# BurryChen/lv_slam

Hardware: AMD Instinct MI355X
Metric: NDT registrations/sec (64k-pt Velodyne pairs) (higher is better)
Workload: dtype f32 terms, f64 accumulation

## Files before the change

lv_slam_amd/csrc/ndt_async.hpp:

```cpp
#pragma once
#include "ndt_types.hpp"
#include "ndt_math.hpp"
#include "ndt_sweep.hpp"
#include "ndt_update.hpp"
#include "ndt_pose_record.hpp"

#define ASYNC_POS_STRIDE 32
#define ASYNC_ARR_STRIDE 16
#define ASYNC_MAX_CTX    4
#define ASYNC_MAX_CARRY  128
#define ASYNC_CTX_SHIFT  24

struct AsyncCtx {
  const float* src; size_t pitch;
  PairState* st; const GridDesc* gd; const BitWord* words; const VoxelRec* recs; const float* cent;
  double* partials; const int* src_cnt; unsigned* arrived; mi355ndt_result* results;
  unsigned* n_done;
  int must_finish;
  int pose_base; PoseRecord* pose; int pose_stride;
  int score_only;
};
struct AsyncTab { AsyncCtx c[ASYNC_MAX_CTX]; };
#define NDT_GP(T) __attribute__((address_space(1))) T*
struct AsyncCtxG {
  NDT_GP(const float) src; size_t pitch;
  NDT_GP(PairState) st; NDT_GP(const GridDesc) gd; NDT_GP(const BitWord) words; NDT_GP(const VoxelRec) recs; NDT_GP(const float) cent;
  NDT_GP(double) partials; NDT_GP(const int) src_cnt; NDT_GP(unsigned) arrived; NDT_GP(mi355ndt_result) results;
  NDT_GP(unsigned) n_done;
  int must_finish;
  int pose_base; NDT_GP(PoseRecord) pose; int pose_stride, score_only;
};
static_assert(sizeof(AsyncCtxG) == sizeof(AsyncCtx) && offsetof(AsyncCtxG, pose) == offsetof(AsyncCtx, pose) && offsetof(AsyncCtxG, n_done) == offsetof(AsyncCtx, n_done),
              "AsyncCtxG mirrors AsyncCtx");
__device__ __forceinline__ AsyncCtx async_ctx_load(const AsyncTab* __restrict__ tab, const int ci) {
  const AsyncCtxG& g = reinterpret_cast<const AsyncCtxG*>(tab->c)[ci];
  AsyncCtx c;
  c.src = (const float*)g.src; c.pitch = g.pitch; c.st = (PairState*)g.st; c.gd = (const GridDesc*)g.gd; c.words = (const BitWord*)g.words;
  c.recs = (const VoxelRec*)g.recs; c.cent = (const float*)g.cent; c.partials = (double*)g.partials; c.src_cnt = (const int*)g.src_cnt;
  c.arrived = (unsigned*)g.arrived; c.results = (mi355ndt_result*)g.results; c.n_done = (unsigned*)g.n_done; c.must_finish = g.must_finish;
  c.pose_base = g.pose_base; c.pose = (PoseRecord*)g.pose; c.pose_stride = g.pose_stride; c.score_only = g.score_only;
  return c;
}
struct CtxStat { unsigned done, total_words, max_cells, plan_exceeded; };
struct StreamStatus { unsigned fin, abort_, n_live, susp; CtxStat ctx[ASYNC_MAX_CTX]; unsigned seq; unsigned pad0_;
                      unsigned long long build_t0, build_t1;
                      unsigned pad_[6]; };
static_assert(sizeof(StreamStatus) == 128, "one status slot is 128 bytes");

struct AsyncCtl {
  unsigned pub;
  unsigned fin;
  unsigned abort_;
  unsigned n_live;
  unsigned susp;
  unsigned pad_[27];
  unsigned pos[8 * ASYNC_POS_STRIDE];
  unsigned carry[ASYNC_MAX_CARRY];
};

#ifndef ASYNC_CLAIM
#define ASYNC_CLAIM(K) ((K) == 1 ? 2 : 1)
#endif
#ifndef ASYNC_HELP_RINGS
#define ASYNC_HELP_RINGS 1
#endif
#define ASYNC_HELP_AFTER 64u
#define ASYNC_SPIN_LIMIT (1u << 18)

NDT_KERNEL void k_async_prepare(const AsyncTab tab, AsyncTab* tab_dev, const int new_ci, const int n_new, PairState* st, const float* __restrict__ guess_cm,
                                const int* __restrict__ src_cnt, const GridDesc* __restrict__ gd, unsigned* arrived, int* active_list, SweepCtl* sweep_ctl ,
                                int* ring, const int ring_cap, AsyncCtl* ctl, const AsyncCtl* prev, unsigned* done_new ,
                                PoseRecord* pose_new , const int pose_cap, unsigned long long* stamp ) {
  const size_t i = (size_t)blockIdx.x * blockDim.x + threadIdx.x;
  if (i == 0 && stamp) *stamp = (unsigned long long)wall_clock64();
  const unsigned nc = prev ? min(prev->susp, (unsigned)ASYNC_MAX_CARRY) : 0u;
  const unsigned n_live = nc + (unsigned)n_new;
  if (i < (size_t)8 * ring_cap) {
    const size_t g = (i % (size_t)ring_cap) * 8 + i / (size_t)ring_cap;
    int w = -1;
    if (g < nc) w = (int)prev->carry[g];
    else if (g < n_live) w = (new_ci << ASYNC_CTX_SHIFT) | (int)(g - nc);
    ring[i] = w;
  }
  if (i < (size_t)n_new * ASYNC_ARR_STRIDE) arrived[i] = 0u;
  if (i < offsetof(AsyncCtl, carry) / sizeof(unsigned)) reinterpret_cast<unsigned*>(ctl)[i] = (i == 0 || i == 3) ? n_live : 0u;
  if (sweep_ctl && i < 2 * sizeof(SweepCtl) / sizeof(int)) reinterpret_cast<int*>(sweep_ctl)[i] = i == 0 ? n_new : 0;
  if (i == 0 && done_new && n_new > 0) *done_new = 0u;
  if (pose_new && i < (size_t)pose_cap) pose_new[i] = pose_record_padding();
  if (i == 0) tab_dev->c[0] = tab.c[0];
  if (i == 1) tab_dev->c[1] = tab.c[1];
  if (i == 2) tab_dev->c[2] = tab.c[2];
  if (i == 3) tab_dev->c[3] = tab.c[3];
  static_assert(ASYNC_MAX_CTX == 4, "the table is copied entry by entry");
  if (i < (size_t)n_new) {
    if (active_list) active_list[i] = (int)i;
    init_pair_state(st[i], guess_cm + i * 16, src_cnt[i], gd[i].status);
  }
}

__device__ __forceinline__ void async_update(const AsyncCtx& C, const int b, const int tw, const int n_pts, const int rows_per_pair, PairState& Ssh, volatile double* sol,
                                             int* ring, const int ring_cap, AsyncCtl* ctl, const unsigned n_live, const int stop_thresh, unsigned long long* hits_total,
                                             const double step_max, const double eps, const int max_iterations, Timeline& tl) {
  PairState* st = C.st;
  const double* partials = C.partials;
  mi355ndt_result* results = C.results;
  const int lane = threadIdx.x & 63;
  __builtin_amdgcn_s_setprio(3);
  gu64* sg = (gu64*)reinterpret_cast<unsigned long long*>(&st[b]);
  unsigned long long* sl = reinterpret_cast<unsigned long long*>(&Ssh);
  state_to_lds<true>(Ssh, &st[b], lane, 64);
  if (lane == 0) sol[6] = 0.0;
  const int nchunks = (n_pts + CHUNK_PTS - 1) / CHUNK_PTS;
  double aw[UPD_WAVES] = {0.0, 0.0, 0.0, 0.0};
  if (lane < NACC) walk_groups<4, true, 2, UPD_WAVES>(partials + (size_t)b * rows_per_pair * NACC + lane, nchunks, 0, 1, aw);
  wave_lds_sync();
  const bool last = __builtin_amdgcn_readfirstlane(Ssh.last_sweep) != 0;
  store_sums(Ssh, lane, wave_sums_total(aw[0], aw[1], aw[2], aw[3]), false, last, hits_total);
  wave_lds_sync();
  TL_STAMP(12);
  constexpr int RB0 = (int)(offsetof(PairState, reb_pn) / 8), RBT = (int)(offsetof(PairState, reb_tag) / 8);
  static_assert(RBT - RB0 == 14, "6 + 8 words of re-basing");
  const bool want_reb = Ssh.phase == PH_STEP;
  bool reb_ok = want_reb && Ssh.reb_tag == (long long)Ssh.sweeps;
  unsigned long long rbw = 0;
  if (reb_ok && lane < 14) rbw = __hip_atomic_load(sg + RB0 + lane, RLX_AGENT);
  if (!last) newton_solve_side(Ssh, sol);
  else if (lane == 0) {
    for (int a = 0; a < 6; a++) sol[a] = 0.0;
    sol[6] = 1.0;
  }
  wave_lds_sync();
  TL_STAMP(13);
  if (want_reb && !reb_ok) {
    unsigned spins = 0;
    while (!reb_ok && spins++ < (1u << 16)) {
      __builtin_amdgcn_s_sleep(2);
      long long tg = 0;
      if (lane == 0) tg = (long long)__hip_atomic_load(sg + RBT, RLX_AGENT);
      reb_ok = __shfl(tg, 0) == (long long)Ssh.sweeps;
    }
    if (reb_ok && lane < 14) rbw = __hip_atomic_load(sg + RB0 + lane, RLX_AGENT);
  }
  if (reb_ok && lane < 14) sl[RB0 + lane] = rbw;
  wave_lds_sync();
  const bool rebased = reb_ok;
  int rc = newton_update(Ssh, &results[b], step_max, eps, max_iterations, 0, sol, rebased, C.score_only != 0);
  rc = __builtin_amdgcn_readfirstlane(rc);
  wave_lds_sync();
  TL_STAMP(14);
  state_from_lds<true>(&st[b], Ssh, lane, 64);
  asm volatile("s_waitcnt vmcnt(0)" ::: "memory");
  if (lane == 0) {
    bool suspend = false;
    if (rc == NEWTON_SWEEP && stop_thresh > 0 && !C.must_finish)
      suspend = n_live - __hip_atomic_load((const gu32*)&ctl->fin, RLX_AGENT) <= (unsigned)stop_thresh;
    if (rc == NEWTON_SWEEP && !suspend) {
      const unsigned g = __hip_atomic_fetch_add((gu32*)&ctl->pub, 1u, RLX_AGENT);
      __hip_atomic_store((gu32*)reinterpret_cast<unsigned*>(ring + (size_t)(g & 7u) * ring_cap + (g >> 3)), (unsigned)tw, RLX_AGENT);
    } else if (rc == NEWTON_SWEEP) {
      const unsigned k = __hip_atomic_fetch_add((gu32*)&ctl->susp, 1u, RLX_AGENT);
      if (k < (unsigned)ASYNC_MAX_CARRY) __hip_atomic_store((gu32*)&ctl->carry[k], (unsigned)tw, RLX_AGENT);
      asm volatile("s_waitcnt vmcnt(0)" ::: "memory");
      __hip_atomic_fetch_add((gu32*)&ctl->fin, 1u, RLX_AGENT);
    } else {
      if (C.pose) C.pose[b] = pose_record(Ssh.final_cm, Ssh.score, Ssh.it, Ssh.converged, C.pose_base + b * C.pose_stride);
      asm volatile("s_waitcnt vmcnt(0)" ::: "memory");
      if (C.n_done) __hip_atomic_fetch_add((gu32*)C.n_done, 1u, RLX_AGENT);
      __hip_atomic_fetch_add((gu32*)&ctl->fin, 1u, RLX_AGENT);
    }
  }
  TL_STAMP(9);
  if (rc == NEWTON_SWEEP) {
    constexpr int RBI = (int)(offsetof(PairState, reb_inc) / 8);
    double pn[6]; float inc[16];
    newton_rebase(Ssh.p, Ssh.dir, Ssh.a_t, pn, inc);
    if (lane == 0) {
      for (int a = 0; a < 6; a++) __hip_atomic_store(sg + RB0 + a, (unsigned long long)__double_as_longlong(pn[a]), RLX_AGENT);
      for (int a = 0; a < 8; a++)
        __hip_atomic_store(sg + RBI + a, (unsigned long long)__float_as_uint(inc[2 * a]) | ((unsigned long long)__float_as_uint(inc[2 * a + 1]) << 32), RLX_AGENT);
      asm volatile("s_waitcnt vmcnt(0)" ::: "memory");
      __hip_atomic_store(sg + RBT, (unsigned long long)(long long)Ssh.sweeps, RLX_AGENT);
    }
  }
  __builtin_amdgcn_s_setprio(0);
}

NDT_KERNEL void k_stream_inputs(const unsigned* __restrict__ host_in, unsigned* __restrict__ dev_in, const unsigned n_in, unsigned* __restrict__ clear, const unsigned n_clear,
                                unsigned long long* stamp) {
  if (threadIdx.x == 0 && stamp) *stamp = (unsigned long long)wall_clock64();
  for (unsigned i = threadIdx.x; i < n_in; i += blockDim.x) dev_in[i] = host_in[i];
  for (unsigned i = threadIdx.x; i < n_clear; i += blockDim.x) clear[i] = 0u;
}

NDT_KERNEL void k_stream_status(const AsyncCtl* __restrict__ ctl, const CtxStat* __restrict__ stat, volatile unsigned* host_slot, const unsigned seq) {
  const int i = threadIdx.x;
  static_assert(offsetof(AsyncCtl, fin) == 4 && offsetof(AsyncCtl, susp) == 16 && offsetof(StreamStatus, ctx) == 16 && offsetof(StreamStatus, seq) == 80 && offsetof(StreamStatus, build_t0) == 88, "status layout");
  if (i < 4) host_slot[i] = reinterpret_cast<const unsigned*>(ctl)[1 + i];
  else if (i < 4 + 4 * ASYNC_MAX_CTX) host_slot[i] = reinterpret_cast<const unsigned*>(stat)[i - 4];
  __threadfence_system();
  __syncthreads();
  if (i == 0) host_slot[20] = seq;
}

#define NDT_CTX_PARAMS(i) const float* __restrict__ src##i, size_t pitch##i, PairState* st##i, const GridDesc* __restrict__ gd##i, const BitWord* __restrict__ words##i, \
                          const VoxelRec* __restrict__ recs##i, double* partials##i, const int* __restrict__ src_cnt##i, unsigned* arrived##i, const float* __restrict__ cent##i
#define NDT_CTX_SEL(f, ci) ((ci) == 0 ? f##0 : (ci) == 1 ? f##1 : (ci) == 2 ? f##2 : f##3)
template <bool PCA, int K, int ORD, bool LEAN = false>
__global__ void __launch_bounds__(SWEEP_THREADS, (SweepTune<PCA, K, ORD, LEAN>::WPE))
k_align_async(const AsyncTab* __restrict__ tab, int items_per_pair, int* ring, int ring_cap, AsyncCtl* ctl, SweepConst sc, unsigned long long* hits_total,
              double step_max, double eps, int max_iterations, int stop_thresh, unsigned debug_abort_pos, unsigned debug_ring_mask, int claim_items,
              NDT_CTX_PARAMS(0), NDT_CTX_PARAMS(1), NDT_CTX_PARAMS(2), NDT_CTX_PARAMS(3)) {
  const int lane = threadIdx.x & 63, wv = threadIdx.x >> 6;
  __shared__ double exp_tab[64];
  __shared__ PairState Ssh[WAVES];
  __shared__ double sol[WAVES][SOL_WORDS];
  if (threadIdx.x < 64) exp_tab[threadIdx.x] = ndtm::c_exp2_64[threadIdx.x];
  __syncthreads();
  const int x = blockIdx.x & 7;
  if (!((debug_ring_mask >> x) & 1u)) return;
  const gu32* ringx = (const gu32*)reinterpret_cast<const unsigned*>(ring + (size_t)x * ring_cap);
  const gu32* fin_p = (const gu32*)&ctl->fin;
  gu32* pos_p = (gu32*)&ctl->pos[x * ASYNC_POS_STRIDE];
  const unsigned n_live = ctl->n_live;
  const int I = items_per_pair;
  const int CLAIM = K == 1 ? ASYNC_CLAIM(1) : (claim_items == 2 ? 2 : 1);
  const int Iu = I / CLAIM;
  Timeline tl;
  auto give_up = [&]() {
    __hip_atomic_store((gu32*)&ctl->abort_, 1u, RLX_AGENT);
    __hip_atomic_store((gu32*)&ctl->fin, n_live, RLX_AGENT);
  };
  bool held = false;
  bool helped = false;
  unsigned held_pos = 0;
  const gu64* pubfin_p = (const gu64*)reinterpret_cast<const unsigned long long*>(ctl);
  static_assert(offsetof(AsyncCtl, pub) == 0 && offsetof(AsyncCtl, fin) == 4, "pub and fin are polled as one 8-byte word");
  auto wait_ticket = [&](unsigned& p, int have) -> int {
    int w = have;
    unsigned sp = p;
    int st = 0;
    if (lane == 0) {
      unsigned spins = helped ? ASYNC_HELP_AFTER : 0u;
      const int t = (int)(p / (unsigned)Iu);
      while (w < 0) {
        const unsigned long long pf = __hip_atomic_load(pubfin_p, RLX_AGENT);
        if ((unsigned)(pf >> 32) >= n_live) { w = -2; break; }
        if (ASYNC_HELP_RINGS && spins >= ASYNC_HELP_AFTER && (spins & 3u) == 3u) {
          const unsigned y = ((unsigned)x + 1u + (spins >> 2) % 7u) & 7u;
          gu32* pos_y = (gu32*)&ctl->pos[y * ASYNC_POS_STRIDE];
          const unsigned q = __hip_atomic_load(pos_y, RLX_AGENT);
          const unsigned pubv = (unsigned)pf;
          const unsigned slots_y = pubv > y ? ((pubv - 1u - y) >> 3) + 1u : 0u;
          const unsigned tq = q / (unsigned)Iu;
          if (tq < slots_y && (int)tq < ring_cap) {
            unsigned expect = q;
            if (__hip_atomic_compare_exchange_strong(pos_y, &expect, q + 1u, __ATOMIC_RELAXED, __ATOMIC_RELAXED, __HIP_MEMORY_SCOPE_AGENT)) {
              const gu32* slot = (const gu32*)reinterpret_cast<const unsigned*>(ring + (size_t)y * ring_cap + tq);
              int ws = (int)__hip_atomic_load(slot, RLX_AGENT);
              unsigned lag = 0;
              while (ws < 0 && ++lag <= ASYNC_SPIN_LIMIT) { __builtin_amdgcn_s_sleep(2); ws = (int)__hip_atomic_load(slot, RLX_AGENT); }
              if (ws < 0) { give_up(); w = -2; break; }
              w = ws; sp = q; st = 1;
              break;
            }
          }
        }
        __builtin_amdgcn_s_sleep(32);
        if (t < ring_cap) w = (int)__hip_atomic_load(ringx + t, RLX_AGENT);
        if (++spins > ASYNC_SPIN_LIMIT) { give_up(); w = -2; break; }
      }
    }
    w = __builtin_amdgcn_readfirstlane(w);
    helped = __builtin_amdgcn_readfirstlane(st) != 0;
    if (helped) { held = true; held_pos = p; p = __builtin_amdgcn_readfirstlane(sp); }
    return w;
  };
  unsigned pos = 0;
  if (lane == 0) pos = __hip_atomic_fetch_add(pos_p, 1u, RLX_AGENT);
  pos = __builtin_amdgcn_readfirstlane(pos);
  int tw = -1;
  if (lane == 0 && (int)(pos / (unsigned)Iu) < ring_cap) tw = (int)__hip_atomic_load(ringx + pos / (unsigned)Iu, RLX_AGENT);
  tw = wait_ticket(pos, tw);
  if (tw < 0) return;
  unsigned pose_w = sweep_pose_words(NDT_CTX_SEL(st, tw >> ASYNC_CTX_SHIFT) + (tw & ((1 << ASYNC_CTX_SHIFT) - 1)));
#pragma unroll 1
  for (;;) {
    if (x == 0 && pos == debug_abort_pos) { if (lane == 0) give_up(); break; }
    const int rem = (int)(pos % (unsigned)Iu) * CLAIM;
    TL_STAMP(10);
    const int ci = tw >> ASYNC_CTX_SHIFT;
    AsyncCtx C = async_ctx_load(tab, ci);
    C.src = NDT_CTX_SEL(src, ci); C.pitch = NDT_CTX_SEL(pitch, ci); C.st = NDT_CTX_SEL(st, ci); C.gd = NDT_CTX_SEL(gd, ci); C.words = NDT_CTX_SEL(words, ci);
    C.recs = NDT_CTX_SEL(recs, ci); C.partials = NDT_CTX_SEL(partials, ci); C.src_cnt = NDT_CTX_SEL(src_cnt, ci); C.arrived = NDT_CTX_SEL(arrived, ci);
    C.cent = NDT_CTX_SEL(cent, ci);
    const int b = tw & ((1 << ASYNC_CTX_SHIFT) - 1);
    const int n_b = C.src_cnt[b];
#ifndef ASYNC_D1_PIPE
#define ASYNC_D1_PIPE 1
#endif
    const bool last = __builtin_amdgcn_readlane(pose_w, POSE_W_LAST) != 0;
    auto items = [&](auto so_c) {
      constexpr bool SO = decltype(so_c)::value;
      if constexpr (K == 1 && ASYNC_D1_PIPE && ORD != 2) {
        sweep_rows_d1<PCA, ORD, ASYNC_CLAIM(1), SO>(b, rem, C.src, C.pitch, C.gd, C.words, C.recs, C.partials, I, sc, exp_tab, pose_w, n_b, b, tl);
      } else {
#pragma unroll 1
        for (int k = 0; k < CLAIM; k++)
          sweep_item<PCA, K, 8, false, ORD, true, SO, 0, LEAN>(b, rem + k, C.src, C.pitch, C.st, C.gd, C.words, C.recs, C.partials, I, sc, C.cent, nullptr, exp_tab, pose_w, n_b, b, tl);
      }
    };
    if (last) items(std::true_type()); else items(std::false_type());
    unsigned npos = held_pos;
    if (lane == 0 && !held) npos = __hip_atomic_fetch_add(pos_p, 1u, RLX_AGENT);
    held = false;
    asm volatile("s_waitcnt vmcnt(0)" ::: "memory");
    npos = __builtin_amdgcn_readfirstlane(npos);
    const int tn = (int)(npos / (unsigned)Iu);
    unsigned old = 0;
    int ntw = -1;
    if (lane == 0) {
      old = __hip_atomic_fetch_add((gu32*)(C.arrived + (size_t)b * ASYNC_ARR_STRIDE), (unsigned)CLAIM, RLX_AGENT);
      if (tn < ring_cap) ntw = (int)__hip_atomic_load(ringx + tn, RLX_AGENT);
    }
    old = __builtin_amdgcn_readfirstlane(old);
    ntw = __builtin_amdgcn_readfirstlane(ntw);
    unsigned npose = 0;
    if (ntw >= 0) npose = sweep_pose_words(NDT_CTX_SEL(st, ntw >> ASYNC_CTX_SHIFT) + (ntw & ((1 << ASYNC_CTX_SHIFT) - 1)));
    TL_STAMP(8);
    if ((old + (unsigned)CLAIM) % (unsigned)I == 0u) {
      async_update(C, b, tw, n_b, I, Ssh[wv], sol[wv], ring, ring_cap, ctl, n_live, stop_thresh, hits_total, step_max, eps, max_iterations, tl);
      TL_STAMP(15);
    }
    if (ntw < 0) {
      ntw = wait_ticket(npos, ntw);
      if (ntw < 0) break;
      npose = sweep_pose_words(NDT_CTX_SEL(st, ntw >> ASYNC_CTX_SHIFT) + (ntw & ((1 << ASYNC_CTX_SHIFT) - 1)));
    }
    tw = ntw; pos = npos; pose_w = npose;
  }
  tl.flush(0, 16);
}
```

lv_slam_amd/csrc/ndt_build.hpp:

```cpp
#pragma once
#include "ndt_types.hpp"
#include "ndt_math.hpp"

__device__ __forceinline__ unsigned mm_enc_max(int ord) { return (unsigned)ord ^ 0x80000000u; }
__device__ __forceinline__ unsigned mm_enc_min(int ord) { return ~((unsigned)ord ^ 0x80000000u); }
__device__ __forceinline__ int mm_dec_max(unsigned e) { return (int)(e ^ 0x80000000u); }
__device__ __forceinline__ int mm_dec_min(unsigned e) { return (int)(~e ^ 0x80000000u); }

#define MM_ILP 3
struct __attribute__((packed, aligned(4))) MmQuad { float v[4]; };
__global__ void __launch_bounds__(256) k_minmax(const float* __restrict__ tgt, size_t pitch, const int* __restrict__ cnt, unsigned* mm) {
  const int b = blockIdx.y;
  const int n = cnt[b];
  const float* X = tgt + (size_t)b * 3 * pitch;
  int mn[3] = {INT_MAX, INT_MAX, INT_MAX}, mx[3] = {INT_MIN, INT_MIN, INT_MIN};
  auto take = [&](const float x, const float y, const float z) {
    if (!finite3(x, y, z)) return;
    const int ox = f2ord(x), oy = f2ord(y), oz = f2ord(z);
    mn[0] = min(mn[0], ox); mx[0] = max(mx[0], ox);
    mn[1] = min(mn[1], oy); mx[1] = max(mx[1], oy);
    mn[2] = min(mn[2], oz); mx[2] = max(mx[2], oz);
  };
  const int stride = (int)(gridDim.x * blockDim.x) * 4;
  for (int i0 = (int)(blockIdx.x * blockDim.x + threadIdx.x) * 4; i0 < n; i0 += stride * MM_ILP) {
    MmQuad qx[MM_ILP], qy[MM_ILP], qz[MM_ILP];
#pragma unroll
    for (int u = 0; u < MM_ILP; u++) {
      const int i = i0 + u * stride;
      if (i + 4 <= n) {
        qx[u] = *reinterpret_cast<const MmQuad*>(X + i); qy[u] = *reinterpret_cast<const MmQuad*>(X + pitch + i);
        qz[u] = *reinterpret_cast<const MmQuad*>(X + 2 * pitch + i);
      } else {
#pragma unroll
        for (int k = 0; k < 4; k++) {
          const bool in = i + k < n;
          qx[u].v[k] = in ? X[i + k] : NAN; qy[u].v[k] = in ? X[pitch + i + k] : NAN; qz[u].v[k] = in ? X[2 * pitch + i + k] : NAN;
        }
      }
    }
#pragma unroll
    for (int u = 0; u < MM_ILP; u++)
#pragma unroll
      for (int k = 0; k < 4; k++) take(qx[u].v[k], qy[u].v[k], qz[u].v[k]);
  }
  __shared__ int red[4][6];
  for (int a = 0; a < 3; a++) {
    for (int o = 32; o > 0; o >>= 1) {
      mn[a] = min(mn[a], __shfl_xor(mn[a], o));
      mx[a] = max(mx[a], __shfl_xor(mx[a], o));
    }
  }
  if ((threadIdx.x & 63) == 0) for (int a = 0; a < 3; a++) { red[threadIdx.x >> 6][a] = mn[a]; red[threadIdx.x >> 6][3 + a] = mx[a]; }
  __syncthreads();
  if (threadIdx.x < 6) {
    const bool is_min = threadIdx.x < 3;
    int v = red[0][threadIdx.x];
    for (int w = 1; w < 4; w++) v = is_min ? min(v, red[w][threadIdx.x]) : max(v, red[w][threadIdx.x]);
    if (is_min) { if (v != INT_MAX) atomicMax(&mm[b * 6 + threadIdx.x], mm_enc_min(v)); }
    else if (v != INT_MIN) atomicMax(&mm[b * 6 + threadIdx.x], mm_enc_max(v));
  }
}

__global__ void k_griddesc(const unsigned* __restrict__ mm, GridDesc* gd, unsigned* nwords, float leaf, int n_pairs, unsigned recs_per_pair) {
  int b = blockIdx.x * blockDim.x + threadIdx.x;
  if (b >= n_pairs) return;
  GridDesc g;
  memset(&g, 0, sizeof g);
  g.leaf = leaf;
  g.inv_leaf = 1.0f / leaf;
  g.rec_off = (unsigned)b * recs_per_pair;
  if (mm[b * 6] == 0u) {
    g.status = GRID_EMPTY;
  } else {
    float mn[3], mx[3];
    for (int a = 0; a < 3; a++) { mn[a] = ord2f(mm_dec_min(mm[b * 6 + a])); mx[a] = ord2f(mm_dec_max(mm[b * 6 + 3 + a])); }
    if (grid_too_big((mx[0] - mn[0]) * g.inv_leaf, (mx[1] - mn[1]) * g.inv_leaf, (mx[2] - mn[2]) * g.inv_leaf)) {
      g.status = GRID_OVERFLOW;
    } else {
      for (int a = 0; a < 3; a++) {
        g.min_b[a] = (int)floorf(mn[a] * g.inv_leaf);
        g.max_b[a] = (int)floorf(mx[a] * g.inv_leaf);
        g.div_b[a] = g.max_b[a] - g.min_b[a] + 1;
      }
      long long nc = (long long)g.div_b[0] * g.div_b[1] * g.div_b[2];
      if (nc > MAX_CELLS) {
        g.status = GRID_CAP;
      } else {
        g.mul1 = g.div_b[0];
        g.mul2 = g.div_b[0] * g.div_b[1];
        g.ncells = (int)nc;
        g.nwords = (int)((nc + 63) >> 6) + 1;
      }
    }
  }
  gd[b] = g;
  nwords[b] = (unsigned)g.nwords;
}

__global__ void __launch_bounds__(1024) k_word_offsets(GridDesc* gd, const unsigned* __restrict__ nwords, int n_pairs, unsigned* out ) {
  __shared__ unsigned sm[17];
  unsigned base = 0, mx = 0;
  for (int b0 = 0; b0 < n_pairs; b0 += 1024) {
    const int b = b0 + threadIdx.x;
    const unsigned v = b < n_pairs ? nwords[b] : 0u;
    unsigned tot;
    const unsigned ex = block_exscan<1024>(v, &tot, sm);
    if (b < n_pairs) { gd[b].word_off = base + ex; mx = max(mx, (unsigned)gd[b].ncells); }
    base += tot;
  }
  if (mx) atomicMax(&out[1], mx);
  if (threadIdx.x == 0) out[0] = base;
}

__global__ void k_build_check(const unsigned* __restrict__ info, GridDesc* gd, unsigned* nwords, int n_pairs, unsigned plan_words, int plan_cb, unsigned* stat ) {
  const int b = blockIdx.x * blockDim.x + threadIdx.x;
  const bool fits = info[0] <= plan_words && (plan_cb >= 31 || info[1] + 1u <= (1u << plan_cb));
  if (b == 0) { stat[0] = info[0]; stat[1] = info[1]; stat[2] = fits ? 0u : 1u; }
  if (fits || b >= n_pairs) return;
  gd[b].status = GRID_CAP; gd[b].ncells = 0; gd[b].nwords = 0; gd[b].word_off = 0; gd[b].n_voxels = 0;
  nwords[b] = 0;
}


#define RUN_ILP 4
template <typename KeyT>
__device__ __forceinline__ void run_heads(const KeyT* __restrict__ K, size_t pitch, size_t i0, size_t stride, int min_points, unsigned cmask,
                                          bool head[RUN_ILP], unsigned cell[RUN_ILP]) {
  KeyT k0[RUN_ILP], km[RUN_ILP], kl[RUN_ILP];
  const size_t span = (size_t)(min_points > 0 ? min_points - 1 : 0);
#pragma unroll
  for (int u = 0; u < RUN_ILP; u++) {
    const size_t i = i0 + (size_t)u * stride;
    const bool in = i < pitch;
    k0[u] = in ? K[i] : (KeyT)cmask;
    km[u] = (in && i != 0) ? K[i - 1] : ~(KeyT)0;
    kl[u] = (in && i + span < pitch) ? K[i + span] : ~(KeyT)0;
  }
#pragma unroll
  for (int u = 0; u < RUN_ILP; u++) {
    const size_t i = i0 + (size_t)u * stride;
    cell[u] = (unsigned)k0[u] & cmask;
    head[u] = i < pitch && cell[u] != cmask && (i == 0 || km[u] != k0[u]) && (i + span < pitch) && kl[u] == k0[u];
  }
}
#define LS_SLICE (64 * RUN_ILP)
static inline unsigned ls_slice_cap(int min_points) { return (unsigned)(LS_SLICE / (min_points > 0 ? min_points : 1) + 2); }
static inline unsigned ls_slices(size_t pitch) { return (unsigned)((pitch + LS_SLICE - 1) / LS_SLICE); }
template <typename KeyT>
__global__ void __launch_bounds__(256) k_mark(const KeyT* __restrict__ keys, size_t pitch, const GridDesc* __restrict__ gd,
                                               BitWord* words, unsigned* heads, unsigned* head_cnt, unsigned n_slices, unsigned slice_cap,
                                               int min_points, int cb) {
  const int b = blockIdx.y;
  const int lane = threadIdx.x & 63;
  const unsigned q = blockIdx.x * 4u + (threadIdx.x >> 6);
  if (q >= n_slices) return;
  const size_t i0 = (size_t)q * LS_SLICE + lane;
  bool head[RUN_ILP];
  unsigned cell[RUN_ILP];
  run_heads<KeyT>(keys + (size_t)b * pitch, pitch, i0, 64, min_points, (1u << cb) - 1u, head, cell);
  unsigned* H = heads + ((size_t)b * n_slices + q) * slice_cap;
  const unsigned long long below = (1ull << lane) - 1ull;
  unsigned n = 0;
#pragma unroll
  for (int u = 0; u < RUN_ILP; u++) {
    const unsigned long long hm = __ballot(head[u]);
    if (head[u]) {
      atomicOr(&words[gd[b].word_off + (cell[u] >> 6)].bits, 1ull << (cell[u] & 63));
      H[n + (unsigned)__popcll(hm & below)] = (unsigned)(i0 + (size_t)u * 64);
    }
    n += (unsigned)__popcll(hm);
  }
  if (lane == 0) head_cnt[(size_t)b * n_slices + q] = n;
}
#define RANK_ROWS 8
#define RANK_WAVES 8
#define RANK_THREADS (64 * RANK_WAVES)
__global__ void __launch_bounds__(RANK_THREADS) k_rank(GridDesc* gd, BitWord* words, const unsigned* __restrict__ heads, const unsigned* __restrict__ head_cnt,
                                                         unsigned n_slices, unsigned slice_cap, unsigned* seg_start) {
  __shared__ unsigned wtot[17];
  static_assert(RANK_WAVES <= 16, "wtot");
  const int b = blockIdx.x;
  BitWord* W = words + gd[b].word_off;
  const int nw = gd[b].nwords;
  const int lane = threadIdx.x & 63, wv = threadIdx.x >> 6;
  unsigned base = 0;
  for (int w0 = 0; w0 < nw; w0 += RANK_THREADS * RANK_ROWS) {
    const int wbase = w0 + wv * 64 * RANK_ROWS;
    unsigned c[RANK_ROWS], ex[RANK_ROWS], run = 0;
#pragma unroll
    for (int u = 0; u < RANK_ROWS; u++) { const int w = wbase + u * 64 + lane; c[u] = (w < nw) ? (unsigned)__popcll(W[w].bits) : 0u; }
#pragma unroll
    for (int u = 0; u < RANK_ROWS; u++) {
      unsigned inc = c[u];
#pragma unroll
      for (int o = 1; o < 64; o <<= 1) { const unsigned t = __shfl_up(inc, o); if (lane >= o) inc += t; }
      ex[u] = run + inc - c[u];
      run += __shfl(inc, 63);
    }
    if (lane == 0) wtot[wv] = run;
    __syncthreads();
    if (wv == 0) {
      const unsigned v = lane < RANK_WAVES ? wtot[lane] : 0u;
      unsigned inc = v;
#pragma unroll
      for (int o = 1; o < RANK_WAVES; o <<= 1) { const unsigned t = __shfl_up(inc, o); if (lane >= o) inc += t; }
      if (lane < RANK_WAVES) wtot[lane] = inc - v;
      if (lane == RANK_WAVES - 1) wtot[16] = inc;
    }
    __syncthreads();
    const unsigned off = base + wtot[wv];
#pragma unroll
    for (int u = 0; u < RANK_ROWS; u++) { const int w = wbase + u * 64 + lane; if (w < nw) W[w].prefix = off + ex[u]; }
    base += wtot[16];
    __syncthreads();
  }
  if (threadIdx.x == 0) gd[b].n_voxels = (int)base;
  unsigned hbase = 0;
  for (unsigned q0 = 0; q0 < n_slices; q0 += RANK_THREADS) {
    const unsigned q = q0 + threadIdx.x;
    const unsigned c = q < n_slices ? head_cnt[(size_t)b * n_slices + q] : 0u;
    unsigned tot;
    const unsigned ex = block_exscan<RANK_THREADS>(c, &tot, wtot);
    const unsigned* H = heads + ((size_t)b * n_slices + q) * slice_cap;
    unsigned* S = seg_start + gd[b].rec_off + hbase + ex;
    for (unsigned k = 0; k < c; k++) S[k] = H[k];
    hbase += tot;
  }
}

__global__ void __launch_bounds__(256) k_sorted_points(const float* __restrict__ tgt, size_t pitch, const unsigned* __restrict__ vals, float4* __restrict__ sorted,
                                                        int nx, int n_targets) {
  int b, bx;
  if (!xcd_map(nx, n_targets, bx, b)) return;
  const float* X = tgt + (size_t)b * 3 * pitch;
  const unsigned* V = vals + (size_t)b * pitch;
  float4* P = sorted + (size_t)b * pitch;
  const size_t i0 = ((size_t)bx * 256 + threadIdx.x);
  const size_t stride = (size_t)nx * 256;
  for (size_t i = i0; i < pitch; i += stride * RUN_ILP) {
    unsigned v[RUN_ILP];
    float4 q[RUN_ILP];
#pragma unroll
    for (int u = 0; u < RUN_ILP; u++) { const size_t j = i + u * stride; v[u] = j < pitch ? V[j] : 0u; }
#pragma unroll
    for (int u = 0; u < RUN_ILP; u++) { const unsigned k = v[u] < pitch ? v[u] : 0u; q[u] = make_float4(X[k], X[pitch + k], X[2 * pitch + k], 0.f); }
#pragma unroll
    for (int u = 0; u < RUN_ILP; u++) { const size_t j = i + u * stride; if (j < pitch) P[j] = q[u]; }
  }
}

#ifdef NDT_TIMELINE
__device__ unsigned long long g_ltl[16];
#define LTL_DECL unsigned long long ltl[12] = {0, 0, 0, 0, 0, 0, 0, 0, 0, 0, 0, 0}; unsigned long long ltl_last = __builtin_readcyclecounter(); const unsigned long long ltl_t0 = ltl_last
#define LTL_STAMP(k) do { __builtin_amdgcn_sched_barrier(0); const unsigned long long t_ = __builtin_readcyclecounter(); ltl[k] += t_ - ltl_last; ltl_last = t_; __builtin_amdgcn_sched_barrier(0); } while (0)
#define LTL_COUNT(k, v) do { ltl[k] += (unsigned long long)(v); } while (0)
#define LTL_FLUSH() do { ltl[10] = 1; ltl[11] = __builtin_readcyclecounter() - ltl_t0; if ((threadIdx.x & 63) == 0 && (blockIdx.x % 24) == (threadIdx.x >> 6) * 5) for (int k_ = 0; k_ < 12; k_++) atomicAdd(&g_ltl[k_], ltl[k_]); } while (0)
#define LTL_ARRIVED1(a) asm volatile("" : "+v"(a))
#else
#define LTL_DECL do {} while (0)
#define LTL_STAMP(k) do {} while (0)
#define LTL_COUNT(k, v) do {} while (0)
#define LTL_FLUSH() do {} while (0)
#define LTL_ARRIVED1(a) do {} while (0)
#endif
#define LS_WAVES 4
template <typename KeyT, bool CENT, bool SORTED = false>
__global__ void __launch_bounds__(64 * LS_WAVES) k_leafsum(const float* __restrict__ tgt, size_t pitch,
                                                           const KeyT* __restrict__ keys, const unsigned* __restrict__ vals ,
                                                           const GridDesc* __restrict__ gd, const unsigned* __restrict__ seg_start,
                                                           double* sums, int* vox_idx, int* vox_n, int cb, float* cent,
                                                           int nx, int n_targets) {
  __shared__ double term[LS_WAVES][64][9];
  __shared__ float termf[CENT ? LS_WAVES : 1][64][3];
  int b, bx;
  if (!xcd_map(nx, n_targets, bx, b)) return;
  const GridDesc& g = gd[b];
  const int lane = threadIdx.x & 63, wv = threadIdx.x >> 6;
  const KeyT* K = keys + (size_t)b * pitch;
  const unsigned* V = vals + (size_t)b * pitch;
  const float* X = tgt + (size_t)b * 3 * pitch;
  const int id0 = bx * LS_WAVES + wv, idstep = nx * LS_WAVES;
  size_t start_next = id0 < g.n_voxels ? seg_start[g.rec_off + id0] : 0;
  LTL_DECL;
  for (int id = id0; id < g.n_voxels; id += idstep) {
    LTL_COUNT(9, 1);
    const size_t start = start_next;
    if (id + idstep < g.n_voxels) start_next = seg_start[g.rec_off + id + idstep];
    double acc = (lane == 3 || lane == 6 || lane == 8) ? 1.0 : 0.0;
    float accf = 0.f;
    int cnt = 0;
    KeyT key = 0;
    for (size_t j0 = start;; j0 += 64) {
      const size_t j = j0 + lane;
      const bool inb = j < pitch;
      const KeyT kj = inb ? K[j] : (KeyT)0;
      float4 pj = make_float4(0.f, 0.f, 0.f, 0.f);
      unsigned pi = 0u;
      if (SORTED) { if (inb) pj = reinterpret_cast<const float4*>(vals)[(size_t)b * pitch + j]; }
      else pi = inb ? V[j] : 0u;
#ifdef NDT_TIMELINE
      { KeyT kq = kj; LTL_ARRIVED1(kq); LTL_ARRIVED1(pi); LTL_ARRIVED1(pj.x); }
      LTL_STAMP(0);
      LTL_COUNT(8, 1);
#endif
      if (j0 == start) key = __shfl(kj, 0);
      const bool in = inb && kj == key;
      const int m = (int)__popcll(__ballot(in));
      if (in) {
        float fx = SORTED ? pj.x : X[pi], fy = SORTED ? pj.y : X[pitch + pi], fz = SORTED ? pj.z : X[2 * pitch + pi];
        LTL_ARRIVED1(fx); LTL_ARRIVED1(fy); LTL_ARRIVED1(fz);
        LTL_STAMP(1);
        const double x = (double)fx, y = (double)fy, z = (double)fz;
        double* t = term[wv][lane];
        t[0] = x; t[1] = y; t[2] = z;
        t[3] = x * x; t[4] = x * y; t[5] = x * z; t[6] = y * y; t[7] = y * z; t[8] = z * z;
        if (CENT) { termf[wv][lane][0] = fx; termf[wv][lane][1] = fy; termf[wv][lane][2] = fz; }
      }
      __builtin_amdgcn_wave_barrier();
      LTL_STAMP(2);
      if (lane < 9) {
        int l = 0;
        for (; l + 8 <= m; l += 8) {
          double t[8];
#pragma unroll
          for (int u = 0; u < 8; u++) t[u] = term[wv][l + u][lane];
#pragma unroll
          for (int u = 0; u < 8; u++) acc += t[u];
        }
        for (; l < m; l++) acc += term[wv][l][lane];
      } else if (CENT && lane < 12) {
        for (int l = 0; l < m; l++) accf += termf[wv][l][lane - 9];
      }
      __builtin_amdgcn_wave_barrier();
      LTL_STAMP(3);
      cnt += m;
      if (m < 64) break;
    }
    if (lane < 9) sums[(size_t)(g.rec_off + id) * 9 + lane] = acc;
    else if (CENT && lane < 12) cent[(size_t)(g.rec_off + id) * 3 + (lane - 9)] = accf / (float)cnt;
    if (lane == 0) {
      vox_idx[g.rec_off + id] = (int)((unsigned)key & ((1u << cb) - 1u));
      vox_n[g.rec_off + id] = cnt;
    }
    LTL_STAMP(4);
  }
  LTL_FLUSH();
}

#ifndef LS_TREE_LEAVES
#define LS_TREE_LEAVES 1
#endif
__global__ void __launch_bounds__(64 * LS_WAVES) k_leafsum_tree(const float* __restrict__ tgt, size_t pitch, const unsigned* __restrict__ keys, const unsigned* __restrict__ vals,
                                                                const GridDesc* __restrict__ gd, const unsigned* __restrict__ seg_start,
                                                                double* sums, int* vox_idx, int* vox_n, int cb, int nx, int n_targets) {
  int b, bx;
  if (!xcd_map(nx, n_targets, bx, b)) return;
  const GridDesc& g = gd[b];
  const int lane = threadIdx.x & 63, wv = threadIdx.x >> 6;
  const unsigned* K = keys + (size_t)b * pitch;
  const unsigned* V = vals + (size_t)b * pitch;
  const float* X = tgt + (size_t)b * 3 * pitch;
  constexpr int NL = LS_TREE_LEAVES;
  const int id0 = bx * LS_WAVES + wv, idstep = nx * LS_WAVES;
  const int nv = g.n_voxels;
  for (int idb = id0; idb < nv; idb += NL * idstep) {
    size_t start[NL];
    bool have[NL];
#pragma unroll
    for (int u = 0; u < NL; u++) { const int id = idb + u * idstep; have[u] = id < nv; start[u] = have[u] ? seg_start[g.rec_off + id] : 0; }
    double a[NL][9];
    int cnt[NL];
    unsigned key[NL];
    bool more[NL];
#pragma unroll
    for (int u = 0; u < NL; u++) {
#pragma unroll
      for (int k = 0; k < 9; k++) a[u][k] = 0.0;
      cnt[u] = 0; key[u] = 0u; more[u] = have[u];
    }
    for (int chunk = 0;; chunk++) {
      bool any = false;
#pragma unroll
      for (int u = 0; u < NL; u++) any = any || more[u];
      if (!any) break;
      unsigned kj[NL], pi[NL];
      bool inb[NL];
#pragma unroll
      for (int u = 0; u < NL; u++) {
        const size_t j = start[u] + (size_t)chunk * 64 + lane;
        inb[u] = more[u] && j < pitch;
        kj[u] = inb[u] ? K[j] : 0u;
        pi[u] = inb[u] ? V[j] : 0u;
      }
      float fx[NL], fy[NL], fz[NL];
      bool in[NL];
#pragma unroll
      for (int u = 0; u < NL; u++) {
        if (chunk == 0) key[u] = __shfl(kj[u], 0);
        in[u] = inb[u] && kj[u] == key[u];
        fx[u] = fy[u] = fz[u] = 0.f;
        if (in[u]) { fx[u] = X[pi[u]]; fy[u] = X[pitch + pi[u]]; fz[u] = X[2 * pitch + pi[u]]; }
      }
#pragma unroll
      for (int u = 0; u < NL; u++) {
        const int m = (int)__popcll(__ballot(in[u]));
        if (in[u]) {
          const double x = (double)fx[u], y = (double)fy[u], z = (double)fz[u];
          a[u][0] += x; a[u][1] += y; a[u][2] += z;
          a[u][3] += x * x; a[u][4] += x * y; a[u][5] += x * z; a[u][6] += y * y; a[u][7] += y * z; a[u][8] += z * z;
        }
        cnt[u] += m;
        more[u] = more[u] && m == 64;
      }
    }
    typedef unsigned int u2v __attribute__((ext_vector_type(2)));
#pragma unroll
    for (int u = 0; u < NL; u++) {
      if (!have[u]) continue;
      const int id = idb + u * idstep;
      double p1[5], p2[3];
#pragma unroll
      for (int i = 0; i < 5; i++) {
        const double x = a[u][i], v = (i + 5 < 9) ? a[u][i + 5] : 0.0;
        const u2v lo = __builtin_amdgcn_permlane32_swap((unsigned)__double2loint(x), (unsigned)__double2loint(v), false, false);
        const u2v hi = __builtin_amdgcn_permlane32_swap((unsigned)__double2hiint(x), (unsigned)__double2hiint(v), false, false);
        p1[i] = __hiloint2double((int)hi.x, (int)lo.x) + __hiloint2double((int)hi.y, (int)lo.y);
      }
#pragma unroll
      for (int i = 0; i < 3; i++) {
        const double x = p1[i], v = (i + 3 < 5) ? p1[i + 3] : 0.0;
        const u2v lo = __builtin_amdgcn_permlane16_swap((unsigned)__double2loint(x), (unsigned)__double2loint(v), false, false);
        const u2v hi = __builtin_amdgcn_permlane16_swap((unsigned)__double2hiint(x), (unsigned)__double2hiint(v), false, false);
        double w = __hiloint2double((int)hi.x, (int)lo.x) + __hiloint2double((int)hi.y, (int)lo.y);
#pragma unroll
        for (int o = 8; o > 0; o >>= 1) w += __shfl_xor(w, o);
        p2[i] = w;
      }
      if ((lane & 15) == 0) {
        const int row = lane >> 4, base = 3 * (row & 1) + 5 * (row >> 1), nrow = (row & 1) ? ((row >> 1) ? 1 : 2) : 3;
        double* o = sums + (size_t)(g.rec_off + id) * 9;
#pragma unroll
        for (int i = 0; i < 3; i++) if (i < nrow) { const int k = base + i; o[k] = p2[i] + ((k == 3 || k == 6 || k == 8) ? 1.0 : 0.0); }
      }
      if (lane == 0) {
        vox_idx[g.rec_off + id] = (int)(key[u] & ((1u << cb) - 1u));
        vox_n[g.rec_off + id] = cnt[u];
      }
    }
  }
}

__global__ void __launch_bounds__(256) k_voxels(const GridDesc* __restrict__ gd, const double* __restrict__ sums,
                                                 VoxelRec* recs, int* vox_n, double eig_mult, int pca, double* icov64, int* kd_weight,
                                                 VoxelRecF* recs_fast ) {
  const int b = blockIdx.y;
  const GridDesc& g = gd[b];
  const int id = blockIdx.x * blockDim.x + threadIdx.x;
  if (id >= g.n_voxels) return;
  const double* A = sums + (size_t)(g.rec_off + id) * 9;
  const double S[3] = {A[0], A[1], A[2]};
  const double C[9] = {A[3], A[4], A[5], A[4], A[6], A[7], A[5], A[7], A[8]};
  const int cnt = vox_n[g.rec_off + id];
  const double dn = (double)cnt;
  double mu[3] = {S[0] / dn, S[1] / dn, S[2] / dn};
  double cov[9];
  for (int a = 0; a < 3; a++)
    for (int c = 0; c < 3; c++) cov[a * 3 + c] = (C[a * 3 + c] - 2 * (S[a] * mu[c])) / dn + mu[a] * mu[c];
  const double f = (dn - 1.0) / dn;
  for (int a = 0; a < 9; a++) cov[a] *= f;
  double ev[3], Vm[9];
  ndtm::eigen_sym3(cov, ev, Vm);
  VoxelRec r;
  r.mean[0] = mu[0]; r.mean[1] = mu[1]; r.mean[2] = mu[2];
  for (int a = 0; a < 9; a++) r.icov[a] = 0.f;
  r.weight = 1;
  int n_out = cnt, kd_w = 0;
  if (ev[0] < 0 || ev[1] < 0 || ev[2] <= 0) {
    n_out = -1;
    r.weight = VOX_DEAD;
    if (icov64) for (int a = 0; a < 9; a++) icov64[(size_t)(g.rec_off + id) * 9 + a] = 0.0;
  } else {
    const double minev = eig_mult * ev[2];
    if (ev[0] < minev) {
      ev[0] = minev;
      if (ev[1] < minev) ev[1] = minev;
      double VD[9], Vi[9];
      for (int a = 0; a < 3; a++) for (int c = 0; c < 3; c++) VD[a * 3 + c] = Vm[a * 3 + c] * ev[c];
      ndtm::mat3_inverse(Vm, Vi);
      ndtm::mat3_mul(VD, Vi, cov);
    }
    if (pca) {
      double s0 = sqrt(ev[0]), s1 = sqrt(ev[1]), s2 = sqrt(ev[2]);
      double f0 = (s2 - s1) / s2, f1 = (s1 - s0) / s2, f2 = s0 / s2;
      int label = 1;
      double fm = f0;
      if (f1 > fm) { fm = f1; label = 2; }
      if (f2 > fm) { label = 3; }
      double scale = (label == 2) ? 1.25 : ((label == 1) ? 0.75 : 1.0);
      double d2d = scale * sqrt((mu[0] * mu[0] + mu[1] * mu[1]) + mu[2] * mu[2]);
      r.weight = (int)d2d;
      kd_w = r.weight;
    }
    double ic[9];
    ndtm::mat3_inverse(cov, ic);
    bool bad = false;
    for (int a = 0; a < 9; a++) { if (!isfinite(ic[a])) bad = true; r.icov[a] = (float)ic[a]; }
    if (bad) { n_out = -1; r.weight = VOX_DEAD; }
    if (icov64) for (int a = 0; a < 9; a++) icov64[(size_t)(g.rec_off + id) * 9 + a] = ic[a];
  }
  recs[g.rec_off + id] = r;
  vox_n[g.rec_off + id] = n_out;
  if (recs_fast) {
    VoxelRecF f;
    for (int a = 0; a < 3; a++) { f.mh[a] = (float)r.mean[a]; f.ml[a] = (float)(r.mean[a] - (double)f.mh[a]); }
    f.c[0] = r.icov[0]; f.c[1] = 0.5f * (r.icov[1] + r.icov[3]); f.c[2] = 0.5f * (r.icov[2] + r.icov[6]);
    f.c[3] = r.icov[4]; f.c[4] = 0.5f * (r.icov[5] + r.icov[7]); f.c[5] = r.icov[8];
    f.pad_[0] = f.pad_[1] = f.pad_[2] = 0.f;
    f.weight = r.weight;
    recs_fast[g.rec_off + id] = f;
  }
  if (kd_weight) kd_weight[g.rec_off + id] = kd_w;
}
```

lv_slam_amd/csrc/ndt_engine.hpp:

```cpp
#pragma once

struct mi355ndt_handle;
struct EngineDel { void operator()(mi355ndt_handle* e) const { (void)mi355ndt_destroy(e); } };

struct StreamCtx {
  long long batch_id = -1; int n_pairs = 0;
  bool busy = false;
  bool redo = false;
  bool done_sync = false;
  long long launch = -1;
  DevBuf<int> d_in; PinBuf<int> h_in; unsigned* h_in_dev = nullptr;
  PinBuf<mi355ndt_result> h_res; mi355ndt_result* d_res_map = nullptr;
  std::vector<float> guesses;
  PoseRecord* d_pose = nullptr; int pose_cap = 0, pose_base = 0, pose_stride = 1;
  std::unique_ptr<mi355ndt_handle, EngineDel> e;
};
struct StreamState {
  static constexpr int EV = 16;
  bool sync_only = false, drop_carry = true;
  int nctx = 0, max_pairs = 0, items = 0, ring_cap = 0, thresh = 0;
  bool thresh_given = false;
  size_t max_tgt = 0, max_src = 0;
  int plan_cb = 0; size_t plan_words = 0;
  void* pose_next = nullptr; size_t pose_cap_next = 0; int pose_base_next = 0, pose_stride_next = 1;
  long long next_id = 0, launches = 0, counted = 0;
  long long recovered_upto = -1;
  DevBuf<AsyncCtl> d_ctl;
  DevBuf<int> d_ring;
  DevBuf<CtxStat> d_stat;
  HipStream build_stream; int reserve_wg = 0, launch_slots = 0;
  bool lean = false;
  bool reserve_given = false;
  int last_reserve = 0, last_slots = 0;
  HipEvent ev_built[ASYNC_MAX_CTX], ev_launched[EV], ev_prepared[EV]; bool prep_first = true;
  PinBuf<volatile StreamStatus> h_status; StreamStatus* d_status = nullptr;
  StreamCtx ctx[ASYNC_MAX_CTX];
};

struct VoxelScratch {
  DevBuf<float> in, x, out;
  DevBuf<unsigned char> keep;
  DevBuf<unsigned> keys, vals;
  DevBuf<unsigned> hist, offs, tmp;
  DevBuf<int> flag, pos;
  DevBuf<int> mm, cnt, aabb, stat;
  DevBuf<PfGrid> grid; DevBuf<McBox> box;
  DevBuf<unsigned char> tab; PinBuf<unsigned char> h_tab;
  DevBuf<double> part; PinBuf<double> h_part;
  PinBuf<int> h_ret;
  bool pending = false;
};

struct CloudIndex {
  static constexpr int NO_INDEX = -1;
  DevBuf<unsigned char> blob; int status = NO_INDEX; int n_fin = 0;
};

struct GicpCache {
  DevBuf<double> cov;
  int k = -1; double eps = 0.0;
};
struct GicpSide {
  DevBuf<float> rows_own; size_t n = 0, pitch = 0;
  int kf_id = -1; bool set = false;
  CloudIndex index; GicpCache cache;
};

struct mi355ndt_handle {
  int device = 0;
  HipStream own_stream;
  hipStream_t stream = nullptr;
  mi355ndt_params prm;
  std::string err;

  int n_pairs = 0, cap_pairs = 0;
  size_t tgt_pitch = 0, src_pitch = 0;
  size_t own_tgt_pitch = 0, own_src_pitch = 0;
  int own_tgt_pairs = 0, own_src_pairs = 0;
  DevBuf<float> d_tgt_own, d_src_own;
  const float *d_tgt = nullptr, *d_src = nullptr;
  DevBuf<int> d_tgt_cnt_own, d_src_cnt_own;
  int *d_tgt_cnt = nullptr, *d_src_cnt = nullptr;
  std::vector<int> h_tgt_cnt, h_src_cnt;
  std::vector<int> up_tgt_cnt, up_src_cnt;
  bool have_target = false, have_source = false;
  GridsBuilt built{};
  bool aligned_once = false;

  unsigned* d_minmax = nullptr;
  DevBuf<GridDesc> d_grid;
  DevBuf<unsigned> d_nwords, d_word_off;
  DevBuf<unsigned> d_keys_a, d_keys_b;
  DevBuf<unsigned> d_vals_a, d_vals_b;
  DevBuf<BitWord> d_words;
  size_t recs_per_pair = 0;
  DevBuf<VoxelRec> d_recs; DevBuf<int> d_vox_idx, d_vox_n;
  DevBuf<unsigned> d_seg_start; DevBuf<double> d_sums;
  DevBuf<unsigned> d_heads, d_head_cnt;
  DevBuf<float> d_cent; DevBuf<double> d_icov64;
  DevBuf<int> d_kdw;
  DevBuf<float4> d_sorted; bool leaf_sorted = false;
  DevBuf<unsigned> d_rs_hist, d_rs_offs;
  DevBuf<double> d_fit;
  DevBuf<BitWord> d_fwords; DevBuf<unsigned> d_fruns;
  DevBuf<int> d_fit_items; DevBuf<float> d_fit_T;
  DevBuf<float> d_pf_out; int pf_count = 0; size_t pf_pitch = 0;
  CloudIndex ol_index; DevBuf<float> d_ol_dist; PinBuf<float> h_ol_dist;
  int ol_cell_mm = 100;
  int pf_group = 0;
  VoxelScratch vs;
  struct Keyframe {
    DevBuf<float> rows; size_t n = 0, pitch = 0; int ch = 3;
    CloudIndex index;
    GicpCache gicp;
  };
  std::map<int, Keyframe> keyframes;
  int kf_next_id = 0;
  int kff_cell_mm = 100;
  struct Gicp {
    mi355ndt_gicp_params prm{20, 1e-3, 2e-3, 5e-4, 200, 20, 5.0};
    GicpSide side[2];
    DevBuf<int> idx, m; DevBuf<double> maha, part; DevBuf<float> moved;
    PinBuf<double> h_rec; double* d_rec = nullptr;
    bool have_corr = false, have_final = false; int n_matched = 0;
    float final_cm[16] = {1,0,0,0, 0,1,0,0, 0,0,1,0, 0,0,0,1};
  } gicp;
  struct GicpBatch {
    struct Slot {
      GicpSide side;
      DevBuf<int> idx; DevBuf<double> maha, part;
      bool have_final = false; float final_cm[16];
    };
    std::vector<Slot> slot;
    DevBuf<int> m;
    PinBuf<double> h_rec; double* d_rec = nullptr;
    PinBuf<GcSlot> h_tab; DevBuf<GcSlot> d_tab;
    int rounds = 0; std::vector<int> requests;
  } gicp_batch;
  struct IcpWork {
    DevBuf<float> W, d2; DevBuf<int> idx; DevBuf<double> part;
    size_t n = 0, pitch = 0;
    bool have_final = false; IcpRun run;
  };
  struct Icp {
    mi355ndt_icp_params prm{0.0, 10, -DBL_MAX, 1.3407807929942596e154, 3, 0};
    GicpSide side[2];
    IcpWork work;
    DevBuf<int> m; DevBuf<float> moved;
    PinBuf<double> h_rec; double* d_rec = nullptr;
  } icp;
  struct IcpBatch {
    struct Slot { GicpSide side; IcpWork work; };
    std::vector<Slot> slot;
    DevBuf<int> m;
    PinBuf<double> h_rec; double* d_rec = nullptr;
    PinBuf<IcpSlot> h_tab; DevBuf<IcpSlot> d_tab;
    int rounds = 0; std::vector<int> requests;
  } icp_batch;
  float last_final[16] = {1,0,0,0, 0,1,0,0, 0,0,1,0, 0,0,0,1};
  PinBuf<unsigned> h_pin_u;

  DevBuf<PairState> d_state;
  DevBuf<double> d_partials;
  int chunks_per_pair = 0;
  int rows_per_pair = 0, pts_per_chunk = CHUNK_PTS;
  int items_per_pair = 0;
  bool async_force = false;
  bool async_align = true;
  int score_only_last = 1;
  DevBuf<int> d_ring; DevBuf<unsigned> d_arrived; DevBuf<AsyncCtl> d_actl;
  PinBuf<AsyncCtl> h_pin_actl;
  DevBuf<AsyncTab> d_atab;
  unsigned debug_abort_pos = 0xFFFFFFFFu;
  unsigned debug_ring_mask = 0xFFu;
  int sweep_waves = 0;
  int last_async_wpe = 0, last_async_grid = 0;
  int arith = 0;
  DevBuf<VoxelRecF> d_recs_fast;
  int pose_model = 0;
  int ndt_class = 0;
  DevBuf<double> d_pcl_rows;
  DevBuf<float> d_euler_rows;
  int f32_sum_order = 0;
  double gauss_last[3] = {0, 0, 0};
  DevBuf<float> d_score_pts; DevBuf<double> d_score_part;
  bool latency_mode = false;
  bool seq_running = false;
  int fine_it = 0;
  int fine_tiles = 2;
  int dyn_shift = -1;
  DevBuf<int> d_grid_of;
  const int* d_grid_of_use = nullptr;
  DevBuf<SeqState> d_seq; DevBuf<mi355ndt_seq_frame> d_seq_out; DevBuf<double> d_stamps;
  PinBuf<volatile int> h_seq_flags; int* d_seq_flags = nullptr;
  DevBuf<float> d_guess_own;
  float* d_guess = nullptr;
  PinBuf<float> h_pin_guess;
  DevBuf<mi355ndt_result> d_results;
  DevBuf<int> d_active;
  DevBuf<int> d_active_list;
  DevBuf<SweepCtl> d_ctl;
  int ctl_idx = 0;
  int n_cu = 256;
  PinBuf<int> h_pin_active;
  HipEvent ev_burst[2];
  DevBuf<unsigned long long> d_hits;
  DevBuf<float> d_hook;
  DevBuf<float> d_aligned;
  PinBuf<float> h_pin_aligned;
  struct UpSlot { PinBuf<float> h; DevBuf<float> d; HipEvent ev; bool used = false, filling = false; };
  static constexpr int UP_SLOTS = 12;
  UpSlot up[UP_SLOTS];
  int up_next = 0;
  static constexpr int UP_STREAMS = 4;
  HipStream copy_stream[UP_STREAMS];
  HipEvent ev_uploads[UP_STREAMS], ev_compute;
  bool uploads_pending = false;
  std::mutex up_mtx;

  bool async_build = false;
  int plan_cb = 0; size_t plan_words = 0;
  unsigned* d_bstat = nullptr;
  bool counts_preloaded = false;
  bool build_stamped = false;
  bool word_off_cleared = false;

  std::unique_ptr<StreamState> ss;
  int s_thresh_opt = -1;
  int s_reserve_opt = -1;

  bool prof = false;
  mi355ndt_profile P{};
  struct EvSpan { hipEvent_t first, second; bool first_shared; };
  std::vector<EvSpan> ev_sweep, ev_update, ev_build;
  hipEvent_t ev_last = nullptr;
  bool ev_last_fresh = false;
  std::vector<hipEvent_t> ev_pool;
  size_t ev_pool_target = 4096;

  ~mi355ndt_handle() {
    for (hipEvent_t e : ev_pool) (void)hipEventDestroy(e);
    for (auto* v : {&ev_sweep, &ev_update, &ev_build})
      for (auto& e : *v) { if (!e.first_shared) (void)hipEventDestroy(e.first); (void)hipEventDestroy(e.second); }
  }
};

#define HIPCHK(h, call)                                                                          \
  do {                                                                                           \
    hipError_t e_ = (call);                                                                      \
    if (e_ != hipSuccess) {                                                                      \
      (h)->err = std::string(#call) + ": " + hipGetErrorString(e_);                              \
      return MI355NDT_ERR_HIP;                                                                   \
    }                                                                                            \
  } while (0)

#define MAX_PAIRS 65535
#ifndef UP_GROUP_PAIRS
#define UP_GROUP_PAIRS 8
#endif
#define UP_GROUP_MAX   (2 * UP_GROUP_PAIRS)
static_assert(UP_GROUP_MAX <= (int)(sizeof(DeintTab::e) / sizeof(DeintTab::e[0])), "k_deinterleave_multi's table");
#define NOT_IN_STREAM(h) do { if ((h)->ss) { (h)->err = "the handle is in stream mode (mi355ndt_stream_begin): call mi355ndt_stream_end first"; return MI355NDT_ERR_STATE; } } while (0)
static inline void cpu_relax() {
#if defined(__x86_64__) || defined(__i386__)
  __builtin_ia32_pause();
#elif defined(__aarch64__)
  asm volatile("yield");
#endif
}
static int ceil_log2(unsigned v) { int b = 0; while ((1u << b) < v) b++; return b; }

static int neighbor_K(int mode) { return mode == MI355NDT_DIRECT1 ? 1 : mode == MI355NDT_DIRECT7 ? 7 : mode == MI355NDT_DIRECT26 ? 26 : 27; }
static void build_offsets(int mode, SweepConst& sc) {
  sc.K = neighbor_K(mode);
  sc.table = sc.K == 1 ? 0 : sc.K == 7 ? 1 : 2;
}

static void gauss_constants3(double outlier_ratio, float resolution, double d[3]) {
  double c1 = 10 * (1 - outlier_ratio);
  double c2 = outlier_ratio / pow((double)resolution, 3);
  d[2] = -log(c2);
  d[0] = -log(c1 + c2) - d[2];
  d[1] = -2 * log((-log(c1 * exp(-0.5) + c2) - d[2]) / d[0]);
}
static void gauss_constants(const mi355ndt_params& p, double& d1, double& d2) {
  double d[3];
  gauss_constants3(p.outlier_ratio, p.resolution, d);
  d1 = d[0]; d2 = d[1];
}

static int check_params(const mi355ndt_params& p) {
  if (!(p.resolution > 0) || !std::isfinite(p.resolution)) return MI355NDT_ERR_BAD_ARG;
  if (p.neighbor_mode < 0 || p.neighbor_mode > 3) return MI355NDT_ERR_BAD_ARG;
  if (p.variant < 0 || p.variant > 1) return MI355NDT_ERR_BAD_ARG;
  if (p.min_points_per_voxel < 1) return MI355NDT_ERR_BAD_ARG;
  if (p.max_iterations < 0) return MI355NDT_ERR_BAD_ARG;
  return MI355NDT_OK;
}

static int eff_model(const mi355ndt_handle* h) { return class_model(h->ndt_class, h->pose_model); }
static GridExtras eff_extras(const mi355ndt_handle* h, bool live = false) { return grid_extras(h->prm, model_arith(h->pose_model, h->arith, h->ndt_class), live, h->ndt_class); }
static bool fast_served(const mi355ndt_handle* h) { return eff_extras(h).recs_fast; }
static float* euler_rows_of(const mi355ndt_handle* h) { return eff_model(h) == POSE_MODEL_EULER ? h->d_euler_rows.p : nullptr; }
static double* pcl_rows_of(const mi355ndt_handle* h) { return h->ndt_class == NDT_CLASS_PCL ? h->d_pcl_rows.p : nullptr; }
#define NOT_EULER(h, what) do { \
    if ((h)->ndt_class == NDT_CLASS_PCL) { (h)->err = what ": not served under MI355NDT_OPT_NDT_CLASS = 1"; return MI355NDT_ERR_UNSUPPORTED; } \
    if ((h)->pose_model == POSE_MODEL_EULER) { (h)->err = what ": not served under MI355NDT_OPT_POSE_MODEL = 1"; return MI355NDT_ERR_UNSUPPORTED; } } while (0)

enum GridWant { GRIDS_ANY, GRIDS_CONFIG, GRIDS_LIVE };
static int ensure_grids(mi355ndt_handle* h, GridWant want);
template <typename N>
static void cloud_changed(mi355ndt_handle* h, bool tgt, int first_pair, int n, const N* counts) {
  std::lock_guard<std::mutex> lk(h->up_mtx);
  std::vector<int>& cnt = tgt ? h->h_tgt_cnt : h->h_src_cnt;
  for (int k = 0; k < n; k++) cnt[(size_t)(first_pair + k)] = (int)counts[k];
  (tgt ? h->have_target : h->have_source) = true;
  if (tgt) h->built.valid = false;
}
static void cloud_changed(mi355ndt_handle* h, bool tgt, int pair, size_t count) { cloud_changed(h, tgt, pair, 1, &count); }
static void clouds_reset(mi355ndt_handle* h, bool tgt, bool src) {
  std::lock_guard<std::mutex> lk(h->up_mtx);
  if (tgt) { std::fill(h->h_tgt_cnt.begin(), h->h_tgt_cnt.end(), 0); h->have_target = false; h->built.valid = false; }
  if (src) { std::fill(h->h_src_cnt.begin(), h->h_src_cnt.end(), 0); h->have_source = false; }
}
static bool async_served(const mi355ndt_handle* h) { return h->async_align && !mt_is_live(h->prm) && !is_pca_kd(h->prm) && model_leaves_rounds(h->pose_model, h->ndt_class); }
static double sweep_alg_bytes(double points, int K) { return points * (12.0 + 4.0 * K); }
static int launch_slots(const mi355ndt_handle* h, const SweepConst& sc, bool fast, bool lean = false) { return h->n_cu * sweep_wpe(sc.K, fast, lean); }
```

lv_slam_amd/csrc/ndt_host_stream.hpp:

```cpp
#pragma once

static void stream_geometry(const StreamState& ss, mi355ndt_handle* e) {
  e->chunks_per_pair = ss.items / QUARTERS; e->rows_per_pair = e->items_per_pair = ss.items; e->pts_per_chunk = CHUNK_PTS; e->fine_it = 0;
}
static size_t stream_partials(const StreamState& ss) { return (size_t)ss.max_pairs * ss.items * NACC; }
static void stream_learn_plan(StreamState& ss, const mi355ndt_handle* e) {
  ss.plan_cb = std::max(ss.plan_cb, e->built.cb);
  ss.plan_words = std::max(ss.plan_words, e->built.total_words + e->built.total_words / 4 + 1024);
}
int mi355ndt_stream_end(mi355ndt_handle* h) {
  if (!h) return MI355NDT_ERR_BAD_HANDLE;
  if (!h->ss) return MI355NDT_OK;
  (void)hipSetDevice(h->device);
  StreamState& ss = *h->ss;
  if (ss.build_stream) (void)hipStreamSynchronize(ss.build_stream);
  (void)hipStreamSynchronize(h->stream);
  for (int c = 0; c < ss.nctx; c++) {
    mi355ndt_handle* e = ss.ctx[c].e.get();
    if (!e) continue;
    ev_collect(e, e->ev_sweep, h->P.sweep_ms, h->P.sweep_launches);
    ev_collect(e, e->ev_update, h->P.update_ms, h->P.update_launches);
    ev_collect(e, e->ev_build, h->P.build_ms, h->P.build_launches);
    h->P.build_alg_bytes += e->P.build_alg_bytes; e->P.build_alg_bytes = 0;
  }
  h->ss.reset();
  return MI355NDT_OK;
}

int mi355ndt_stream_begin(mi355ndt_handle* h, int n_contexts, int max_pairs, size_t max_tgt, size_t max_src) {
  if (!h) return MI355NDT_ERR_BAD_HANDLE;
  if (n_contexts < 2 || n_contexts > ASYNC_MAX_CTX || max_pairs < 1 || max_pairs > MAX_PAIRS || max_pairs >= (1 << ASYNC_CTX_SHIFT) ||
      max_tgt == 0 || max_src == 0 || max_tgt >= (1u << 31) || max_src >= (1u << 31)) return MI355NDT_ERR_BAD_ARG;
  if (h->ss) return MI355NDT_ERR_STATE;
  NOT_EULER(h, "mi355ndt_stream_begin");
  HIPCHK(h, hipSetDevice(h->device));
  HIPCHK(h, hipStreamSynchronize(h->stream));
  std::unique_ptr<StreamState> session(new StreamState());
  StreamState& ss = *session;
  ss.nctx = n_contexts; ss.max_pairs = max_pairs; ss.max_tgt = max_tgt; ss.max_src = max_src;
  ss.items = std::max(1, (int)((max_src + CHUNK_PTS - 1) / CHUNK_PTS)) * QUARTERS;
  ss.sync_only = !async_served(h);
  h->built = GridsBuilt{};
  SweepConst sc;
  make_sweep_const(h, sc);
  const int slots = launch_slots(h, sc, fast_served(h));
  {
    const int iu = ss.items / (sc.K == 1 ? ASYNC_CLAIM(1) : sc.K == 7 ? 2 : 1);
    const int waves = slots * WAVES;
    int t = h->s_thresh_opt >= 0 ? h->s_thresh_opt : 4 * ((waves + iu - 1) / std::max(1, iu));
    const char* env = std::getenv("MI355NDT_STREAM_THRESH");
    if (env) t = std::atoi(env);
    ss.thresh = std::max(0, std::min(t, ASYNC_MAX_CARRY));
    ss.thresh_given = h->s_thresh_opt >= 0 || env;
  }
  {
    const bool small_batch = (unsigned long long)max_pairs * (unsigned long long)max_tgt <= 768ull * 65536ull;
    int r = sc.K == 1 ? (max_tgt <= 98304 ? 128 : 96) : ((sc.K == 7 && small_batch) ? (sc.pca ? 32 : 64) : 0);
    if (const char* e = std::getenv("MI355NDT_STREAM_RESERVE")) { r = std::atoi(e); ss.reserve_given = true; }
    if (h->s_reserve_opt >= 0) { r = h->s_reserve_opt; ss.reserve_given = true; }
    r = std::max(0, std::min(r, slots / 2)) & ~7;
    if (n_contexts < 3) r = 0;
    ss.reserve_wg = r;
    ss.launch_slots = std::max(8, slots - r);
    ss.last_reserve = r; ss.last_slots = ss.launch_slots;
  }
  ss.ring_cap = async_ring_cap(h, (long long)max_pairs + ASYNC_MAX_CARRY);
  if (ss.ring_cap == 0) ss.sync_only = true;
  if (ss.d_stat.realloc_exact(ASYNC_MAX_CTX) != hipSuccess ||
      hipMemsetAsync(ss.d_stat, 0, ASYNC_MAX_CTX * sizeof(CtxStat), h->stream) != hipSuccess) return MI355NDT_ERR_HIP;
  for (int c = 0; c < n_contexts; c++) {
    StreamCtx& S = ss.ctx[c];
    mi355ndt_handle* e = nullptr;
    int rc = mi355ndt_create(&h->prm, h->device, &e);
    S.e.reset(e);
    if (rc) return rc;
    if (ss.reserve_wg > 0 && !ss.build_stream) {
      if (ss.build_stream.create() != hipSuccess) return MI355NDT_ERR_HIP;
      for (auto& ev : ss.ev_built) if (ev.create() != hipSuccess) return MI355NDT_ERR_HIP;
      for (auto& ev : ss.ev_launched) if (ev.create() != hipSuccess) return MI355NDT_ERR_HIP;
      for (auto& ev : ss.ev_prepared) if (ev.create() != hipSuccess) return MI355NDT_ERR_HIP;
      if (const char* pf = std::getenv("MI355NDT_STREAM_PREP_FIRST")) ss.prep_first = std::atoi(pf) != 0;
    }
    rc = mi355ndt_set_stream(e, ss.reserve_wg > 0 ? ss.build_stream : h->stream);
    if (rc) return rc;
    e->sweep_waves = h->sweep_waves; e->f32_sum_order = h->f32_sum_order; e->arith = h->arith; e->async_align = h->async_align; e->dyn_shift = h->dyn_shift; e->score_only_last = h->score_only_last;
    e->async_build = true;
    e->ev_pool_target = 128;
    rc = ensure_pair_arrays(e, max_pairs);
    if (rc) { h->err = e->err; return rc; }
    static_assert(sizeof(float) == sizeof(int), "the input block holds ints and floats");
    const size_t in_words = (size_t)max_pairs * (2 + 16);
    if (S.d_in.realloc_exact(in_words) != hipSuccess || S.h_in.realloc_exact(in_words, hipHostMallocMapped) != hipSuccess ||
        !(S.h_in_dev = (unsigned*)S.h_in.dev()) ||
        S.h_res.realloc_exact(max_pairs, hipHostMallocMapped | hipHostMallocCoherent) != hipSuccess ||
        !(S.d_res_map = S.h_res.dev())) { h->err = "stream_begin: allocation failed"; return MI355NDT_ERR_HIP; }
    e->d_tgt_cnt = S.d_in; e->d_src_cnt = S.d_in + max_pairs; e->d_guess = (float*)(S.d_in + 2 * (size_t)max_pairs);
    e->d_bstat = reinterpret_cast<unsigned*>(ss.d_stat + c);
    if (e->d_partials.reserve(stream_partials(ss)) != hipSuccess || e->d_arrived.reserve((size_t)max_pairs * ASYNC_ARR_STRIDE) != hipSuccess)
      { h->err = "stream_begin: allocation failed"; return MI355NDT_ERR_HIP; }
    if (h->prof) (void)mi355ndt_profile_enable(e, 1);
  }
  if (ss.d_ctl.realloc_exact(2) != hipSuccess || hipMemsetAsync(ss.d_ctl, 0, 2 * sizeof(AsyncCtl), h->stream) != hipSuccess ||
      ss.h_status.realloc_exact(StreamState::EV, hipHostMallocMapped | hipHostMallocCoherent) != hipSuccess ||
      !(ss.d_status = ss.h_status.dev())) return MI355NDT_ERR_HIP;
  memset((void*)ss.h_status.p, 0, StreamState::EV * sizeof(StreamStatus));
  if (h->d_atab.reserve(1) != hipSuccess) return MI355NDT_ERR_HIP;
  if (!ss.sync_only && ss.d_ring.realloc_exact((size_t)8 * ss.ring_cap) != hipSuccess) { (void)hipGetLastError(); ss.sync_only = true; }
  if (ss.build_stream) HIPCHK(h, hipStreamSynchronize(ss.build_stream));
  HIPCHK(h, hipStreamSynchronize(h->stream));
  h->ss = std::move(session);
  return MI355NDT_OK;
}

static int stream_launch(mi355ndt_handle* h, int new_ci, int n_new) {
  StreamState& ss = *h->ss;
  hipStream_t s = h->stream;
  SweepConst sc;
  make_sweep_const(h, sc);
  AsyncLaunch L;
  memset(&L.tab, 0, sizeof L.tab);
  const bool flush = new_ci < 0;
  for (int c = 0; c < ss.nctx; c++) {
    mi355ndt_handle* e = ss.ctx[c].e.get();
    if (!e->d_src) continue;
    fill_async_ctx(e, L.tab.c[c]);
    L.tab.c[c].results = ss.ctx[c].d_res_map;
    L.tab.c[c].n_done = &ss.d_stat[c].done;
    L.tab.c[c].pose = ss.ctx[c].busy ? ss.ctx[c].d_pose : nullptr; L.tab.c[c].pose_base = ss.ctx[c].pose_base; L.tab.c[c].pose_stride = ss.ctx[c].pose_stride;
    const int ahead = (ss.reserve_wg > 0 || ss.nctx >= 3) ? 2 : 1;
    bool mf = flush;
    for (int a = 1; a <= ahead; a++) mf = mf || c == (new_ci + a) % ss.nctx;
    L.tab.c[c].must_finish = mf ? 1 : 0;
  }
  const long long j = ss.launches;
  L.new_ci = flush ? 0 : new_ci; L.n_new = flush ? 0 : n_new;
  if (!flush) {
    mi355ndt_handle* e = ss.ctx[new_ci].e.get();
    L.st_new = e->d_state; L.guess_new = e->d_guess; L.src_cnt_new = e->d_src_cnt; L.gd_new = e->d_grid; L.arrived_new = e->d_arrived;
    L.active_list = e->d_active_list; L.sweep_ctl = nullptr; L.done_new = &ss.d_stat[new_ci].done;
    L.pose_new = ss.ctx[new_ci].d_pose; L.pose_cap = ss.ctx[new_ci].pose_cap;
  }
  L.tab_dev = h->d_atab; L.ring = ss.d_ring; L.ring_cap = ss.ring_cap;
  L.ctl = ss.d_ctl + (j & 1); L.prev = ss.drop_carry ? nullptr : ss.d_ctl + ((j + 1) & 1);
  L.items_per_pair = ss.items; L.stop_thresh = flush ? 0 : (ss.thresh_given ? ss.thresh : std::min(ss.thresh, n_new / 4)); L.debug_abort_pos = h->debug_abort_pos; L.debug_ring_mask = h->debug_ring_mask;
  if (!flush) {
    const mi355ndt_handle* e = ss.ctx[new_ci].e.get();
    const int tgt_max = *std::max_element(e->h_tgt_cnt.begin(), e->h_tgt_cnt.begin() + n_new);
    ss.lean = async_lean(h, sc, sweep_ord(h, sc), tgt_max > 0 ? (size_t)tgt_max : ss.max_tgt);
  }
  L.lean = ss.lean;
  L.reserve_wg = flush ? 0 : ss.reserve_wg;
  if (L.lean && !flush && !ss.reserve_given && ss.reserve_wg > 0) L.reserve_wg = LEAN_RESERVE_WG;
  if (L.lean) L.reserve_wg = std::min(L.reserve_wg, launch_slots(h, sc, false, true) / 2) & ~7;
  L.ev_prepared = (ss.reserve_wg > 0 && ss.prep_first) ? ss.ev_prepared[j % StreamState::EV] : nullptr;
  L.claim_items = (sc.K == 7 && L.stop_thresh > 0) ? 2 : 1;
  h->ev_last_fresh = false;
  if (!flush && ss.reserve_wg > 0) HIPCHK(h, hipStreamWaitEvent(s, ss.ev_built[new_ci], 0));
  L.stamp_end = (!flush && h->prof) ? &ss.d_status[j % StreamState::EV].build_t1 : nullptr;
  int rc = launch_async(h, sc, L);
  if (rc) return rc;
  ss.drop_carry = false;
  if (!flush) { ss.last_reserve = L.reserve_wg; ss.last_slots = h->last_async_grid; }
  const int slot = (int)(j % StreamState::EV);
  k_stream_status<<<1, 64, 0, s>>>(L.ctl, ss.d_stat, reinterpret_cast<volatile unsigned*>(ss.d_status + slot), (unsigned)(j + 1));
  HIPCHK(h, hipGetLastError());
  if (ss.reserve_wg > 0) HIPCHK(h, hipEventRecord(ss.ev_launched[slot], s));
  ss.launches++;
  h->P.stream_launches++;
  return MI355NDT_OK;
}

static int stream_wait_launch(mi355ndt_handle* h, long long j) {
  StreamState& ss = *h->ss;
  volatile StreamStatus* st = ss.h_status + (j % StreamState::EV);
  const auto t0 = std::chrono::steady_clock::now();
  for (unsigned spins = 0; st->seq != (unsigned)(j + 1); spins++) {
    if ((spins & 1023) == 1023) {
      if (std::chrono::steady_clock::now() - t0 > std::chrono::seconds(60)) { h->err = "stream: the device stopped reporting"; return MI355NDT_ERR_STATE; }
      std::this_thread::yield();
    } else cpu_relax();
  }
  std::atomic_thread_fence(std::memory_order_acquire);
  for (; ss.counted <= j; ss.counted++) {
    volatile StreamStatus* c = ss.h_status + (ss.counted % StreamState::EV);
    h->P.stream_carried += c->susp;
    const unsigned long long b0 = c->build_t0, b1 = c->build_t1;
    if (b0 && b1 > b0) { h->P.build_ms += (double)(b1 - b0) * 1e-5; h->P.build_launches++; }
    c->build_t0 = 0; c->build_t1 = 0;
  }
  return MI355NDT_OK;
}

static int stream_run_sync(mi355ndt_handle* h, StreamCtx& S) {
  StreamState& ss = *h->ss;
  mi355ndt_handle* e = S.e.get();
  if (ss.build_stream) HIPCHK(h, hipStreamSynchronize(ss.build_stream));
  HIPCHK(h, hipStreamSynchronize(h->stream));
  e->async_build = false; e->counts_preloaded = false;
  e->up_tgt_cnt.clear(); e->up_src_cnt.clear();
  int rc = mi355ndt_batch_build_targets(e);
  if (rc == MI355NDT_OK) rc = mi355ndt_batch_align(e, S.guesses.data(), S.h_res);
  e->async_build = true;
  if (rc) { h->err = e->err; return rc; }
  stream_learn_plan(ss, e);
  stream_geometry(ss, e);
  if (e->d_partials.reserve(stream_partials(ss)) != hipSuccess) return MI355NDT_ERR_HIP;
  return MI355NDT_OK;
}

int mi355ndt_stream_submit(mi355ndt_handle* h, int n_pairs, const float* d_t, const int* tc, size_t tp, const float* d_s, const int* scnt, size_t sp,
                           const float* guesses, long long* batch_id) {
  if (!h) return MI355NDT_ERR_BAD_HANDLE;
  if (!h->ss) return MI355NDT_ERR_STATE;
  StreamState& ss = *h->ss;
  if (n_pairs < 1 || n_pairs > ss.max_pairs || !guesses || !batch_id || !tc || !scnt) return MI355NDT_ERR_BAD_ARG;
  HIPCHK(h, hipSetDevice(h->device));
  const long long id = ss.next_id;
  const int ci = (int)(id % ss.nctx);
  StreamCtx& S = ss.ctx[ci];
  if (S.busy) { h->err = "stream_submit: collect batch " + std::to_string(S.batch_id) + " first (its context is the one this batch needs)"; return MI355NDT_ERR_STATE; }
  mi355ndt_handle* e = S.e.get();
  for (int b = 0; b < n_pairs; b++) if ((size_t)scnt[b] > (size_t)(ss.items / QUARTERS) * CHUNK_PTS) return MI355NDT_ERR_BAD_ARG;
  int rc = mi355ndt_batch_bind_device(e, n_pairs, d_t, tc, tp, d_s, scnt, sp);
  if (rc) { h->err = e->err; return rc; }
  e->prm = h->prm;
  S.batch_id = id; S.n_pairs = n_pairs; S.redo = false; S.done_sync = false; S.launch = -1;
  S.guesses.assign(guesses, guesses + (size_t)n_pairs * 16);
  S.d_pose = (PoseRecord*)ss.pose_next; S.pose_cap = (int)ss.pose_cap_next; S.pose_base = ss.pose_base_next; S.pose_stride = ss.pose_stride_next;
  ss.pose_next = nullptr; ss.pose_cap_next = 0;
  if (S.d_pose && (size_t)n_pairs > (size_t)S.pose_cap) return MI355NDT_ERR_BAD_ARG;
  if (ss.sync_only) {
    rc = stream_run_sync(h, S);
    if (rc) return rc;
    S.done_sync = true; S.busy = true;
    *batch_id = id; ss.next_id++;
    return MI355NDT_OK;
  }
  memcpy(S.h_in, tc, (size_t)n_pairs * sizeof(int));
  memcpy(S.h_in + ss.max_pairs, scnt, (size_t)n_pairs * sizeof(int));
  memcpy(S.h_in + 2 * (size_t)ss.max_pairs, guesses, (size_t)n_pairs * 16 * sizeof(float));
  if (ss.reserve_wg > 0 && ss.prep_first && ss.launches >= 1)
    HIPCHK(h, hipStreamWaitEvent(e->stream, ss.ev_prepared[(ss.launches - 1) % StreamState::EV], 0));
  else if (ss.reserve_wg > 0 && ss.launches >= 2)
    HIPCHK(h, hipStreamWaitEvent(e->stream, ss.ev_launched[(ss.launches - 2) % StreamState::EV], 0));
  k_stream_inputs<<<1, 1024, 0, e->stream>>>(S.h_in_dev, reinterpret_cast<unsigned*>(S.d_in.p), (unsigned)(2 * (size_t)ss.max_pairs + (size_t)n_pairs * 16),
                                            e->d_word_off, (unsigned)(2 + 6 * (size_t)e->cap_pairs),
                                            h->prof ? &ss.d_status[ss.launches % StreamState::EV].build_t0 : nullptr);
  e->word_off_cleared = true;
  e->build_stamped = h->prof;
  e->counts_preloaded = true; e->up_src_cnt.clear(); e->up_tgt_cnt.clear();
  e->async_build = true;
  e->plan_cb = ss.plan_cb; e->plan_words = ss.plan_words;
  HIPCHK(h, e->d_words.reserve(e->plan_words));
  rc = mi355ndt_batch_build_targets(e);
  if (rc) { h->err = e->err; return rc; }
  if (!(e->plan_cb > 0 && e->plan_words > 0)) stream_learn_plan(ss, e);
  if (ss.reserve_wg > 0) HIPCHK(h, hipEventRecord(ss.ev_built[ci], e->stream));
  stream_geometry(ss, e);
  gauss_constants3(h->prm.outlier_ratio, h->prm.resolution, h->gauss_last);
  S.busy = true;
  S.launch = ss.launches;
  rc = stream_launch(h, ci, n_pairs);
  if (rc) {
    ss.sync_only = true;
    rc = stream_run_sync(h, S);
    if (rc) { S.busy = false; return rc; }
    S.done_sync = true;
  }
  e->aligned_once = true;
  *batch_id = id; ss.next_id++;
  return MI355NDT_OK;
}

int mi355ndt_stream_submit_host(mi355ndt_handle* h, int n_pairs, const void* const* targets, const size_t* target_counts, const void* const* sources,
                                const size_t* source_counts, size_t stride, const float* guesses, int n_threads, long long* batch_id) {
  if (!h) return MI355NDT_ERR_BAD_HANDLE;
  if (!h->ss) return MI355NDT_ERR_STATE;
  StreamState& ss = *h->ss;
  if (n_pairs < 1 || n_pairs > ss.max_pairs || !targets || !target_counts || !sources || !source_counts || stride < 12 || !guesses || !batch_id) return MI355NDT_ERR_BAD_ARG;
  for (int b = 0; b < n_pairs; b++)
    if (target_counts[b] > ss.max_tgt || source_counts[b] > ss.max_src || (!targets[b] && target_counts[b]) || (!sources[b] && source_counts[b])) return MI355NDT_ERR_BAD_ARG;
  HIPCHK(h, hipSetDevice(h->device));
  const int ci = (int)(ss.next_id % ss.nctx);
  StreamCtx& S = ss.ctx[ci];
  if (S.busy) { h->err = "stream_submit_host: collect batch " + std::to_string(S.batch_id) + " first (its context is the one this batch needs)"; return MI355NDT_ERR_STATE; }
  mi355ndt_handle* e = S.e.get();
  const size_t tp = (ss.max_tgt + 63) & ~(size_t)63, sp = (ss.max_src + 63) & ~(size_t)63;
  if (!e->d_tgt_own || !e->d_src_own || e->own_tgt_pairs < ss.max_pairs || e->own_src_pairs < ss.max_pairs || e->own_tgt_pitch != tp || e->own_src_pitch != sp) {
    int rc = mi355ndt_batch_reserve(e, ss.max_pairs, ss.max_tgt, ss.max_src);
    if (rc) { h->err = e->err; return rc; }
  }
  e->n_pairs = ss.max_pairs; e->d_tgt = e->d_tgt_own; e->d_src = e->d_src_own; e->tgt_pitch = tp; e->src_pitch = sp;
  int rc = mi355ndt_batch_set_clouds(e, 0, n_pairs, targets, target_counts, sources, source_counts, stride, n_threads);
  if (rc) { h->err = e->err; return rc; }
  std::vector<int> tc((size_t)n_pairs), sc((size_t)n_pairs);
  for (int b = 0; b < n_pairs; b++) { tc[(size_t)b] = (int)target_counts[b]; sc[(size_t)b] = (int)source_counts[b]; }
  return mi355ndt_stream_submit(h, n_pairs, e->d_tgt_own, tc.data(), tp, e->d_src_own, sc.data(), sp, guesses, batch_id);
}

int mi355ndt_stream_pose_records(mi355ndt_handle* h, void* d_records, size_t capacity, int id_base, int id_stride) {
  if (!h) return MI355NDT_ERR_BAD_HANDLE;
  if (!h->ss) return MI355NDT_ERR_STATE;
  if ((d_records && capacity == 0) || capacity > (size_t)MAX_PAIRS) return MI355NDT_ERR_BAD_ARG;
  StreamState& ss = *h->ss;
  ss.pose_next = d_records; ss.pose_cap_next = d_records ? capacity : 0; ss.pose_base_next = id_base; ss.pose_stride_next = id_stride;
  return MI355NDT_OK;
}

static void stream_recover(mi355ndt_handle* h) {
  StreamState& ss = *h->ss;
  if (ss.build_stream) (void)hipStreamSynchronize(ss.build_stream);
  (void)hipStreamSynchronize(h->stream);
  CtxStat st[ASYNC_MAX_CTX];
  if (hipMemcpy(st, ss.d_stat, sizeof st, hipMemcpyDeviceToHost) != hipSuccess) memset(st, 0, sizeof st);
  for (int c = 0; c < ss.nctx; c++) {
    StreamCtx& S = ss.ctx[c];
    if (S.busy && !S.done_sync && st[c].done != (unsigned)S.n_pairs) S.redo = true;
  }
  ss.drop_carry = true;
  ss.recovered_upto = ss.launches - 1;
  h->P.async_fallbacks++;
}

int mi355ndt_stream_collect(mi355ndt_handle* h, long long batch_id, mi355ndt_result* out) {
  if (!h) return MI355NDT_ERR_BAD_HANDLE;
  if (!h->ss) return MI355NDT_ERR_STATE;
  StreamState& ss = *h->ss;
  if (batch_id < 0 || batch_id >= ss.next_id || !out) return MI355NDT_ERR_BAD_ARG;
  HIPCHK(h, hipSetDevice(h->device));
  const int ci = (int)(batch_id % ss.nctx);
  StreamCtx& S = ss.ctx[ci];
  if (!S.busy || S.batch_id != batch_id) return MI355NDT_ERR_BAD_ARG;
  mi355ndt_handle* e = S.e.get();
  bool reran = S.done_sync;
  if (!S.done_sync) {
    long long j = S.launch;
    bool plan_exceeded = false;
    for (;;) {
      int rc = stream_wait_launch(h, j);
      if (rc) return rc;
      const StreamStatus st = *const_cast<const StreamStatus*>(ss.h_status + (j % StreamState::EV));
      if (st.abort_ && !S.redo && j > ss.recovered_upto) stream_recover(h);
      plan_exceeded = st.ctx[ci].plan_exceeded != 0;
      if (S.redo || plan_exceeded) break;
      if (st.ctx[ci].done == (unsigned)S.n_pairs) break;
      if (j + 1 < ss.launches) { j++; continue; }
      rc = stream_launch(h, -1, 0);
      if (rc) { stream_recover(h); S.redo = true; break; }
      j = ss.launches - 1;
    }
    if (S.redo || plan_exceeded) {
      const int rc = stream_run_sync(h, S);
      if (rc) { S.busy = false; return rc; }
      h->P.stream_redone++;
      reran = true;
    }
  }
  if (S.d_pose && reran) {
    int rc = mi355ndt_batch_pose_records(e, S.pose_base, S.pose_stride, S.d_pose, (size_t)S.pose_cap);
    if (rc) { h->err = e->err; return rc; }
  }
  memcpy(out, S.h_res, (size_t)S.n_pairs * sizeof(mi355ndt_result));
  tolerance_warnings(h, out, S.n_pairs);
  account_sweeps(h, out, e->h_src_cnt.data(), S.n_pairs, neighbor_K(h->prm.neighbor_mode));
  S.busy = false;
  return MI355NDT_OK;
}

int mi355ndt_pack_pose_records(const mi355ndt_result* results, int n, int id_base, int id_stride, void* records, size_t capacity) {
  if (!results || !records || n < 0 || (size_t)n > capacity) return MI355NDT_ERR_BAD_ARG;
  PoseRecord* out = (PoseRecord*)records;
  for (size_t k = 0; k < capacity; k++) {
    PoseRecord r;
    memset(&r, 0, sizeof r);
    r.pair_id = -1;
    if (k < (size_t)n) {
      for (int a = 0; a < 16; a++) r.final_cm[a] = results[k].final_colmajor[a];
      r.score = (float)results[k].score;
      r.iterations = results[k].iterations;
      r.converged = results[k].converged;
      r.pair_id = id_base + (int)k * id_stride;
    }
    out[k] = r;
  }
  return MI355NDT_OK;
}
```

lv_slam_amd/csrc/ndt_host_sweep.hpp:

```cpp
#pragma once

#include "ndt_sweep_exists.hpp"
template <int N> using IC = std::integral_constant<int, N>;
template <class F>
static int dispatch_sweep(bool pca, int K, int ord, int it, F&& f) {
  int rc = MI355NDT_ERR_UNSUPPORTED;
  auto one = [&](auto P, auto KK, auto O, auto IT) {
    if constexpr (sweep_exists(decltype(P)::value, decltype(KK)::value, decltype(O)::value, decltype(IT)::value))
      if (pca == decltype(P)::value && K == decltype(KK)::value && ord == decltype(O)::value && it == decltype(IT)::value) rc = f(P, KK, O, IT);
  };
  auto by_it = [&](auto P, auto KK, auto O) { one(P, KK, O, IC<SWEEP_IT_BATCH>{}); one(P, KK, O, IC<1>{}); one(P, KK, O, IC<2>{}); };
  auto by_ord = [&](auto P, auto KK) { by_it(P, KK, IC<0>{}); by_it(P, KK, IC<1>{}); by_it(P, KK, IC<2>{}); };
  auto by_K = [&](auto P) { by_ord(P, IC<1>{}); by_ord(P, IC<7>{}); by_ord(P, IC<26>{}); by_ord(P, IC<27>{}); };
  by_K(std::false_type{}); by_K(std::true_type{});
  return rc;
}

static_assert(sizeof(VoxelRec) == LEAN_REC_BYTES, "the record the estimate counts");
static bool async_lean(const mi355ndt_handle* h, const SweepConst& sc, int ord, size_t tgt_pts) {
  return async_served(h) && lean_exists(sc.pca != 0, sc.K, ord) && sweep_waves_choice(h->sweep_waves, h->prm, ord, tgt_pts) == 3;
}
constexpr int LEAN_RESERVE_WG = 96;

static int prep_align_ws(mi355ndt_handle* h) {
  const int B = h->n_pairs;
  int maxn = 0;
  for (int b = 0; b < B; b++) maxn = std::max(maxn, h->h_src_cnt[b]);
  h->chunks_per_pair = std::max(1, (maxn + CHUNK_PTS - 1) / CHUNK_PTS);
  {
    const bool fine_served = sweep_exists(false, neighbor_K(h->prm.neighbor_mode), 0, h->fine_tiles);
    const bool small = h->seq_running || (long long)B * h->chunks_per_pair * QUARTERS < 4LL * h->n_cu * WAVES;
    h->fine_it = (h->latency_mode && fine_served && !mt_is_live(h->prm) && small && model_leaves_rounds(h->pose_model, h->ndt_class)) ? h->fine_tiles : 0;
  }
  if (eff_model(h) == POSE_MODEL_EULER) HIPCHK(h, h->d_euler_rows.reserve((size_t)B * EULER_ROW_WORDS));
  if (h->ndt_class == NDT_CLASS_PCL) HIPCHK(h, h->d_pcl_rows.reserve((size_t)B * EULER_ROW_WORDS));
  if (h->fine_it) {
    const int item_pts = h->fine_it * 64;
    h->pts_per_chunk = 4 * item_pts;
    h->rows_per_pair = std::max(1, (maxn + h->pts_per_chunk - 1) / h->pts_per_chunk);
    h->items_per_pair = 4 * h->rows_per_pair;
  } else {
    h->rows_per_pair = h->chunks_per_pair * QUARTERS;
    h->items_per_pair = h->rows_per_pair;
    h->pts_per_chunk = CHUNK_PTS;
  }
  size_t need = (size_t)B * std::max(h->rows_per_pair, h->chunks_per_pair * QUARTERS) * NACC;
  HIPCHK(h, h->d_partials.reserve(need));
  if (h->up_src_cnt.size() != (size_t)B || !std::equal(h->up_src_cnt.begin(), h->up_src_cnt.end(), h->h_src_cnt.begin())) {
    HIPCHK(h, hipMemcpyAsync(h->d_src_cnt, h->h_src_cnt.data(), B * sizeof(int), hipMemcpyHostToDevice, h->stream));
    HIPCHK(h, hipStreamSynchronize(h->stream));
    h->up_src_cnt.assign(h->h_src_cnt.begin(), h->h_src_cnt.begin() + B);
  }
  return MI355NDT_OK;
}

static void make_sweep_const(const mi355ndt_handle* h, SweepConst& sc) {
  double d1, d2;
  gauss_constants(h->prm, d1, d2);
  sc.d1 = d1;
  sc.d2f = (float)d2;
  sc.pca = h->prm.variant == MI355NDT_VARIANT_PCA;
  const float leaf = (h->built.valid && h->built.leaf > 0.f) ? h->built.leaf : h->prm.resolution;
  { int ex; float mant = std::frexp(leaf, &ex); sc.leaf_pow2 = (mant == 0.5f) && ex > -100 && ex < 100; sc.inv_leaf = 1.0f / leaf; }
  sc.kd_r2 = (float)((double)h->prm.resolution * (double)h->prm.resolution);
  build_offsets(class_neighbor_mode(h->ndt_class, h->prm.neighbor_mode), sc);
  sc.dyn_shift = h->dyn_shift >= 0 ? h->dyn_shift : (sc.K == 1 ? 3 : 2);
  sc.host_flags = nullptr;
  sc.seq_no = 0;
  sc.rebase_block = 0;
  sc.d1f = (float)d1;
  sc.kq = (float)(-0.5 * (double)sc.d2f * 1.4426950408889634);
  sc.euler_rows = euler_rows_of(h);
  sc.pcl_rows = pcl_rows_of(h);
  sc.icov64 = h->d_icov64.p;
  sc.d2 = d2;
}

static int sweep_ord(const mi355ndt_handle* h, const SweepConst& sc) {
  if (h->ndt_class == NDT_CLASS_PCL) return 0;
  if (fast_served(h) && (h->built.made.recs_fast || h->ss)) return 2;
  return h->f32_sum_order;
}
static const VoxelRec* sweep_recs(const mi355ndt_handle* h, const SweepConst& sc) {
  return sweep_ord(h, sc) == 2 ? reinterpret_cast<const VoxelRec*>(h->d_recs_fast.p) : h->d_recs;
}

template <int K>
static void launch_sweep_euler_k(mi355ndt_handle* h, const SweepConst& sc, int ord, dim3 grid, SweepCtl* ctl, SweepCtl* ctl_next) {
  auto kern = ord == 1 ? k_sweep<false, K, SWEEP_IT_BATCH, false, 1, 1> : k_sweep<false, K, SWEEP_IT_BATCH, false, 0, 1>;
  kern<<<grid, SWEEP_THREADS, 0, h->stream>>>(h->d_src, h->src_pitch, h->d_state, h->d_grid, h->d_words, h->d_recs, h->d_partials, h->items_per_pair, h->d_active_list, ctl,
                                              ctl_next, sc, h->d_cent, h->d_grid_of_use);
}
static int launch_sweep_euler(mi355ndt_handle* h, const SweepConst& sc, int ord, dim3 grid, SweepCtl* ctl, SweepCtl* ctl_next) {
  if (sc.pca || h->fine_it || !euler_sweep_exists(sc.K, ord) || !sc.euler_rows) return MI355NDT_ERR_UNSUPPORTED;
  if (sc.K == 1) launch_sweep_euler_k<1>(h, sc, ord, grid, ctl, ctl_next);
  else if (sc.K == 7) launch_sweep_euler_k<7>(h, sc, ord, grid, ctl, ctl_next);
  else if (sc.K == 26) launch_sweep_euler_k<26>(h, sc, ord, grid, ctl, ctl_next);
  else launch_sweep_euler_k<27>(h, sc, ord, grid, ctl, ctl_next);
  return MI355NDT_OK;
}

static int launch_sweep(mi355ndt_handle* h, const SweepConst& sc, int max_pairs = -1) {
  const int ord = sweep_ord(h, sc);
  dim3 grid((unsigned)launch_slots(h, sc, ord == 2));
  if (h->prof) HIPCHK(h, ev_begin(h, h->ev_sweep));
  SweepCtl *ctl = h->d_ctl + h->ctl_idx, *ctl_next = h->d_ctl + (h->ctl_idx ^ 1);
  if (h->fine_it) {
    const long long items = (long long)(max_pairs > 0 ? max_pairs : h->n_pairs) * h->items_per_pair;
    grid.x = (unsigned)std::max(1LL, std::min((long long)grid.x, (items + WAVES - 1) / WAVES));
    if (sc.rebase_block) grid.x += 1;
  }
  if (h->ndt_class == NDT_CLASS_PCL) {
    if (sc.pca || h->fine_it || sc.K != 27 || !sc.pcl_rows || !sc.icov64 || !h->built.made.icov64 || !h->built.made.cent) {
      h->err = "no sweep kernel serves this configuration under MI355NDT_OPT_NDT_CLASS = 1";
      return MI355NDT_ERR_UNSUPPORTED;
    }
    k_sweep<false, 27, SWEEP_IT_BATCH, false, 0, 2><<<grid, SWEEP_THREADS, 0, h->stream>>>(h->d_src, h->src_pitch, h->d_state, h->d_grid, h->d_words, h->d_recs, h->d_partials,
                                                                                           h->items_per_pair, h->d_active_list, ctl, ctl_next, sc, h->d_cent, h->d_grid_of_use);
  } else if (h->pose_model == POSE_MODEL_EULER) {
    const int rc = launch_sweep_euler(h, sc, ord, grid, ctl, ctl_next);
    if (rc) { h->err = "no sweep kernel serves this configuration under MI355NDT_OPT_POSE_MODEL = 1"; return rc; }
  } else if (!h->fine_it && sc.pca && sc.K == 27) {
    const dim3 kdgrid((unsigned)h->chunks_per_pair, (unsigned)h->n_pairs);
    auto kd = ord == 1 ? k_sweep_pca_kd<1> : k_sweep_pca_kd<0>;
    kd<<<kdgrid, SWEEP_THREADS, 0, h->stream>>>(h->d_src, h->src_pitch, h->d_state, h->d_grid, h->d_words, h->d_recs, h->d_cent, h->d_kdw, h->d_partials,
                                                h->chunks_per_pair, h->d_active_list, ctl, ctl_next, sc);
  } else {
    const int rc = dispatch_sweep(sc.pca != 0, sc.K, ord, h->fine_it ? h->fine_it : SWEEP_IT_BATCH, [&](auto P, auto KK, auto O, auto IT) {
      constexpr int it = decltype(IT)::value;
      k_sweep<decltype(P)::value, decltype(KK)::value, it, it != SWEEP_IT_BATCH, decltype(O)::value><<<grid, SWEEP_THREADS, 0, h->stream>>>(
          h->d_src, h->src_pitch, h->d_state, h->d_grid, h->d_words, sweep_recs(h, sc), h->d_partials, h->items_per_pair, h->d_active_list, ctl, ctl_next, sc,
          h->d_cent, h->d_grid_of_use);
      return MI355NDT_OK;
    });
    if (rc) { h->err = "no sweep kernel serves this configuration"; return rc; }
  }
  h->ctl_idx ^= 1;
  if (h->prof) HIPCHK(h, ev_end(h, h->ev_sweep));
  return MI355NDT_OK;
}

static void launch_hessian(mi355ndt_handle* h, const SweepConst& sc) {
  double gc[3] = {0, 0, 0};
  gauss_constants(h->prm, gc[0], gc[1]);
  k_hessian<<<dim3((unsigned)h->chunks_per_pair, (unsigned)h->n_pairs), HESS_THREADS, 0, h->stream>>>(
      h->d_src, h->src_pitch, h->d_state, h->d_grid, h->d_words, h->d_recs, h->d_icov64, h->d_cent, h->d_partials, h->chunks_per_pair,
      gc[0], gc[1], sc.kd_r2, sc.leaf_pow2, sc.inv_leaf);
}


struct AsyncLaunch {
  AsyncTab tab;
  int new_ci = 0, n_new = 0;
  PairState* st_new = nullptr; const float* guess_new = nullptr; const int* src_cnt_new = nullptr; const GridDesc* gd_new = nullptr; unsigned* arrived_new = nullptr;
  int* active_list = nullptr; SweepCtl* sweep_ctl = nullptr; unsigned* done_new = nullptr; PoseRecord* pose_new = nullptr; int pose_cap = 0;
  AsyncTab* tab_dev = nullptr; int* ring = nullptr; int ring_cap = 0; AsyncCtl* ctl = nullptr; const AsyncCtl* prev = nullptr;
  int items_per_pair = 0, stop_thresh = 0; unsigned debug_abort_pos = 0xFFFFFFFFu, debug_ring_mask = 0xFFu;
  unsigned long long* stamp_end = nullptr;
  int claim_items = 1;
  int reserve_wg = 0;
  bool lean = false;
  hipEvent_t ev_prepared = nullptr;
};
#define NDT_CTX_ARGS(i) L.tab.c[i].src, L.tab.c[i].pitch, L.tab.c[i].st, L.tab.c[i].gd, L.tab.c[i].words, L.tab.c[i].recs, L.tab.c[i].partials, L.tab.c[i].src_cnt, \
                        L.tab.c[i].arrived, L.tab.c[i].cent
template <bool PCA, int K, int ORD, bool LEAN = false>
static int launch_async_t(mi355ndt_handle* h, const SweepConst& sc, const AsyncLaunch& L) {
  auto kern = k_align_async<PCA, K, ORD, LEAN>;
  static std::atomic<int> per_cu_of_device[64];
  int per_cu = per_cu_of_device[h->device & 63].load(std::memory_order_relaxed);
  if (per_cu == 0) {
    if (hipOccupancyMaxActiveBlocksPerMultiprocessor(&per_cu, kern, SWEEP_THREADS, 0) != hipSuccess) { (void)hipGetLastError(); return MI355NDT_ERR_UNSUPPORTED; }
    per_cu_of_device[h->device & 63].store(per_cu, std::memory_order_relaxed);
  }
  const int slots = launch_slots(h, sc, ORD == 2, LEAN);
  if (per_cu * h->n_cu < slots || slots < 8) return MI355NDT_ERR_UNSUPPORTED;
  dim3 grid((unsigned)std::max(8, slots - L.reserve_wg));
  kern<<<grid, SWEEP_THREADS, 0, h->stream>>>(L.tab_dev, L.items_per_pair, L.ring, L.ring_cap, L.ctl, sc, h->prof ? h->d_hits : nullptr,
                                             h->prm.step_size, h->prm.trans_epsilon, h->prm.max_iterations, L.stop_thresh, L.debug_abort_pos, L.debug_ring_mask, L.claim_items,
                                             NDT_CTX_ARGS(0), NDT_CTX_ARGS(1), NDT_CTX_ARGS(2), NDT_CTX_ARGS(3));
  h->last_async_wpe = SweepTune<PCA, K, ORD, LEAN>::WPE; h->last_async_grid = (int)grid.x;
  return MI355NDT_OK;
}
static int launch_async(mi355ndt_handle* h, const SweepConst& sc, const AsyncLaunch& L) {
  hipStream_t s = h->stream;
  {
    const size_t n = std::max(std::max(std::max((size_t)8 * L.ring_cap, (size_t)L.n_new * ASYNC_ARR_STRIDE), sizeof(AsyncCtl) / sizeof(unsigned)), (size_t)L.pose_cap);
    k_async_prepare<<<(unsigned)((n + 255) / 256), 256, 0, s>>>(L.tab, L.tab_dev, L.new_ci, L.n_new, L.st_new, L.guess_new, L.src_cnt_new, L.gd_new, L.arrived_new,
                                                               L.active_list, L.sweep_ctl, L.ring, L.ring_cap, L.ctl, L.prev, L.done_new, L.pose_new, L.pose_cap, L.stamp_end);
    if (L.ev_prepared) HIPCHK(h, hipEventRecord(L.ev_prepared, s));
  }
  if (h->prof) HIPCHK(h, ev_begin(h, h->ev_sweep));
  const int rc = dispatch_sweep(sc.pca != 0, sc.K, sweep_ord(h, sc), SWEEP_IT_BATCH, [&](auto P, auto KK, auto O, auto) {
    if constexpr (lean_exists(decltype(P)::value, decltype(KK)::value, decltype(O)::value))
      if (L.lean) return launch_async_t<false, 7, decltype(O)::value, true>(h, sc, L);
    return launch_async_t<decltype(P)::value, decltype(KK)::value, decltype(O)::value>(h, sc, L);
  });
  if (h->prof) HIPCHK(h, ev_end(h, h->ev_sweep));
  return rc;
}
static int async_ring_cap(const mi355ndt_handle* h, long long pairs) {
  const long long cap = (pairs * ((long long)h->prm.max_iterations + 4) + 7) / 8 + 1;
  return cap > (1LL << 26) ? 0 : (int)cap;
}
static void fill_async_ctx(const mi355ndt_handle* e, AsyncCtx& c) {
  SweepConst sc;
  make_sweep_const(e, sc);
  c.src = e->d_src; c.pitch = e->src_pitch; c.st = e->d_state; c.gd = e->d_grid; c.words = e->d_words; c.recs = sweep_recs(e, sc); c.cent = e->d_cent;
  c.partials = e->d_partials; c.src_cnt = e->d_src_cnt; c.arrived = e->d_arrived; c.results = e->d_results; c.n_done = nullptr; c.must_finish = 1; c.pose = nullptr; c.pose_base = 0; c.pose_stride = 0; c.score_only = e->score_only_last;
}
```

Before: 70100.

## Move async prep to build stream and fold status reporting into sweep kernel

The per-launch prepare kernel now runs on the context's build stream instead of the sweep stream. Carried-over pairs are adopted into the ring by the sweep kernel itself at entry, rather than copied during prepare. The separate status kernel is removed, and the last finishing workgroup writes the host status slot. Control, ring and table sets grow from 2 to 4, and input staging spins on an 'entered' flag rather than on events. Together this removes two kernel launches and the event dependencies between launches, letting prepare overlap the previous sweep, at the cost of more memory and device-side spin-waits. k_voxels also gets a minimum-blocks launch bound.

```diff
diff --git a/lv_slam_amd/csrc/ndt_async.hpp b/lv_slam_amd/csrc/ndt_async.hpp
--- a/lv_slam_amd/csrc/ndt_async.hpp
+++ b/lv_slam_amd/csrc/ndt_async.hpp
@@ -44,7 +44,8 @@
 struct CtxStat { unsigned done, total_words, max_cells, plan_exceeded; };
 struct StreamStatus { unsigned fin, abort_, n_live, susp; CtxStat ctx[ASYNC_MAX_CTX]; unsigned seq; unsigned pad0_;
                       unsigned long long build_t0, build_t1;
-                      unsigned pad_[6]; };
+                      unsigned long long launch_t0, launch_t1;
+                      unsigned pad_[2]; };
 static_assert(sizeof(StreamStatus) == 128, "one status slot is 128 bytes");
 
 struct AsyncCtl {
@@ -53,10 +54,18 @@
   unsigned abort_;
   unsigned n_live;
   unsigned susp;
-  unsigned pad_[27];
+  unsigned adopt;
+  unsigned entered;
+  unsigned seq;
+  const AsyncCtl* prev;
+  StreamStatus* report;
+  const CtxStat* stat;
+  unsigned prof;
+  unsigned pad_[17];
   unsigned pos[8 * ASYNC_POS_STRIDE];
   unsigned carry[ASYNC_MAX_CARRY];
 };
+static_assert(offsetof(AsyncCtl, pos) == 128 && offsetof(AsyncCtl, prev) == 32, "the control words are one 128-byte line");
 
 #ifndef ASYNC_CLAIM
 #define ASYNC_CLAIM(K) ((K) == 1 ? 2 : 1)
@@ -70,20 +79,22 @@
 NDT_KERNEL void k_async_prepare(const AsyncTab tab, AsyncTab* tab_dev, const int new_ci, const int n_new, PairState* st, const float* __restrict__ guess_cm,
                                 const int* __restrict__ src_cnt, const GridDesc* __restrict__ gd, unsigned* arrived, int* active_list, SweepCtl* sweep_ctl ,
                                 int* ring, const int ring_cap, AsyncCtl* ctl, const AsyncCtl* prev, unsigned* done_new ,
-                                PoseRecord* pose_new , const int pose_cap, unsigned long long* stamp ) {
+                                PoseRecord* pose_new , const int pose_cap, unsigned long long* stamp ,
+                                StreamStatus* report , const CtxStat* stat, const unsigned seq, const unsigned prof) {
   const size_t i = (size_t)blockIdx.x * blockDim.x + threadIdx.x;
   if (i == 0 && stamp) *stamp = (unsigned long long)wall_clock64();
-  const unsigned nc = prev ? min(prev->susp, (unsigned)ASYNC_MAX_CARRY) : 0u;
-  const unsigned n_live = nc + (unsigned)n_new;
   if (i < (size_t)8 * ring_cap) {
     const size_t g = (i % (size_t)ring_cap) * 8 + i / (size_t)ring_cap;
-    int w = -1;
-    if (g < nc) w = (int)prev->carry[g];
-    else if (g < n_live) w = (new_ci << ASYNC_CTX_SHIFT) | (int)(g - nc);
-    ring[i] = w;
+    ring[i] = g < (size_t)n_new ? ((new_ci << ASYNC_CTX_SHIFT) | (int)g) : -1;
   }
   if (i < (size_t)n_new * ASYNC_ARR_STRIDE) arrived[i] = 0u;
-  if (i < offsetof(AsyncCtl, carry) / sizeof(unsigned)) reinterpret_cast<unsigned*>(ctl)[i] = (i == 0 || i == 3) ? n_live : 0u;
+  constexpr size_t HDR = offsetof(AsyncCtl, pos) / sizeof(unsigned);
+  if (i >= HDR && i < offsetof(AsyncCtl, carry) / sizeof(unsigned)) reinterpret_cast<unsigned*>(ctl)[i] = 0u;
+  if (i == 0) {
+    ctl->pub = ctl->n_live = (unsigned)n_new;
+    ctl->fin = ctl->abort_ = ctl->susp = ctl->adopt = ctl->entered = 0u;
+    ctl->seq = seq; ctl->prev = prev; ctl->report = report; ctl->stat = stat; ctl->prof = prof;
+  }
   if (sweep_ctl && i < 2 * sizeof(SweepCtl) / sizeof(int)) reinterpret_cast<int*>(sweep_ctl)[i] = i == 0 ? n_new : 0;
   if (i == 0 && done_new && n_new > 0) *done_new = 0u;
   if (pose_new && i < (size_t)pose_cap) pose_new[i] = pose_record_padding();
@@ -96,6 +107,23 @@
     if (active_list) active_list[i] = (int)i;
     init_pair_state(st[i], guess_cm + i * 16, src_cnt[i], gd[i].status);
   }
+}
+
+static __device__ __noinline__ void async_report(AsyncCtl* ctl, const unsigned n_live, const int lane) {
+  static_assert(offsetof(AsyncCtl, fin) == 4 && offsetof(AsyncCtl, susp) == 16 && offsetof(StreamStatus, ctx) == 16 && offsetof(StreamStatus, seq) == 80 &&
+                offsetof(StreamStatus, build_t0) == 88 && sizeof(CtxStat) == 16, "status layout");
+  unsigned* slot = reinterpret_cast<unsigned*>(ctl->report);
+  if (!slot) return;
+  asm volatile("s_waitcnt vmcnt(0)" ::: "memory");
+  unsigned v = 0u;
+  if (lane < 4) v = __hip_atomic_load((const gu32*)reinterpret_cast<const unsigned*>(ctl) + 1 + lane, RLX_AGENT);
+  else if (lane < 4 + 4 * ASYNC_MAX_CTX) v = __hip_atomic_load((const gu32*)reinterpret_cast<const unsigned*>(ctl->stat) + (lane - 4), RLX_AGENT);
+  if (lane == 2) v = n_live;
+  if (lane < 4 + 4 * ASYNC_MAX_CTX) __hip_atomic_store(slot + lane, v, __ATOMIC_RELAXED, __HIP_MEMORY_SCOPE_SYSTEM);
+  if (lane == 0 && ctl->prof)
+    __hip_atomic_store(&ctl->report->launch_t1, (unsigned long long)wall_clock64(), __ATOMIC_RELAXED, __HIP_MEMORY_SCOPE_SYSTEM);
+  asm volatile("s_waitcnt vmcnt(0)" ::: "memory");
+  if (lane == 0) __hip_atomic_store(slot + offsetof(StreamStatus, seq) / sizeof(unsigned), ctl->seq, __ATOMIC_RELAXED, __HIP_MEMORY_SCOPE_SYSTEM);
 }
 
 __device__ __forceinline__ void async_update(const AsyncCtx& C, const int b, const int tw, const int n_pts, const int rows_per_pair, PairState& Ssh, volatile double* sol,
@@ -150,6 +178,7 @@
   TL_STAMP(14);
   state_from_lds<true>(&st[b], Ssh, lane, 64);
   asm volatile("s_waitcnt vmcnt(0)" ::: "memory");
+  int ended = 0;
   if (lane == 0) {
     bool suspend = false;
     if (rc == NEWTON_SWEEP && stop_thresh > 0 && !C.must_finish)
@@ -161,14 +190,19 @@
       const unsigned k = __hip_atomic_fetch_add((gu32*)&ctl->susp, 1u, RLX_AGENT);
       if (k < (unsigned)ASYNC_MAX_CARRY) __hip_atomic_store((gu32*)&ctl->carry[k], (unsigned)tw, RLX_AGENT);
       asm volatile("s_waitcnt vmcnt(0)" ::: "memory");
-      __hip_atomic_fetch_add((gu32*)&ctl->fin, 1u, RLX_AGENT);
+      ended = __hip_atomic_fetch_add((gu32*)&ctl->fin, 1u, RLX_AGENT) + 1u == n_live;
     } else {
       if (C.pose) C.pose[b] = pose_record(Ssh.final_cm, Ssh.score, Ssh.it, Ssh.converged, C.pose_base + b * C.pose_stride);
       asm volatile("s_waitcnt vmcnt(0)" ::: "memory");
-      if (C.n_done) __hip_atomic_fetch_add((gu32*)C.n_done, 1u, RLX_AGENT);
-      __hip_atomic_fetch_add((gu32*)&ctl->fin, 1u, RLX_AGENT);
-    }
-  }
+      if (C.n_done) {
+        __builtin_amdgcn_fence(__ATOMIC_RELEASE, "");
+        __hip_atomic_fetch_add((gu32*)C.n_done, 1u, RLX_AGENT);
+        asm volatile("s_waitcnt vmcnt(0)" ::: "memory");
+      }
+      ended = __hip_atomic_fetch_add((gu32*)&ctl->fin, 1u, RLX_AGENT) + 1u == n_live;
+    }
+  }
+  if (__builtin_amdgcn_readfirstlane(ended)) async_report(ctl, n_live, lane);
   TL_STAMP(9);
   if (rc == NEWTON_SWEEP) {
     constexpr int RBI = (int)(offsetof(PairState, reb_inc) / 8);
@@ -186,20 +220,34 @@
 }
 
 NDT_KERNEL void k_stream_inputs(const unsigned* __restrict__ host_in, unsigned* __restrict__ dev_in, const unsigned n_in, unsigned* __restrict__ clear, const unsigned n_clear,
-                                unsigned long long* stamp) {
+                                unsigned long long* stamp, const unsigned* launch_in) {
+  if (launch_in) {
+    if (threadIdx.x == 0)
+      for (unsigned spins = 0; __hip_atomic_load((const gu32*)launch_in, RLX_AGENT) == 0u && spins < ASYNC_SPIN_LIMIT; spins++) __builtin_amdgcn_s_sleep(32);
+    __syncthreads();
+  }
   if (threadIdx.x == 0 && stamp) *stamp = (unsigned long long)wall_clock64();
   for (unsigned i = threadIdx.x; i < n_in; i += blockDim.x) dev_in[i] = host_in[i];
   for (unsigned i = threadIdx.x; i < n_clear; i += blockDim.x) clear[i] = 0u;
 }
 
-NDT_KERNEL void k_stream_status(const AsyncCtl* __restrict__ ctl, const CtxStat* __restrict__ stat, volatile unsigned* host_slot, const unsigned seq) {
-  const int i = threadIdx.x;
-  static_assert(offsetof(AsyncCtl, fin) == 4 && offsetof(AsyncCtl, susp) == 16 && offsetof(StreamStatus, ctx) == 16 && offsetof(StreamStatus, seq) == 80 && offsetof(StreamStatus, build_t0) == 88, "status layout");
-  if (i < 4) host_slot[i] = reinterpret_cast<const unsigned*>(ctl)[1 + i];
-  else if (i < 4 + 4 * ASYNC_MAX_CTX) host_slot[i] = reinterpret_cast<const unsigned*>(stat)[i - 4];
-  __threadfence_system();
-  __syncthreads();
-  if (i == 0) host_slot[20] = seq;
+__device__ __forceinline__ unsigned async_enter(AsyncCtl* ctl, int* ring, const int ring_cap) {
+  const AsyncCtl* prev = ctl->prev;
+  const unsigned n_carry = prev ? min(prev->susp, (unsigned)ASYNC_MAX_CARRY) : 0u;
+  if (threadIdx.x == 0) {
+    if (ctl->prof && ctl->report) {
+      if (__hip_atomic_fetch_add((gu32*)&ctl->entered, 1u, RLX_AGENT) == 0u)
+        __hip_atomic_store(&ctl->report->launch_t0, (unsigned long long)wall_clock64(), __ATOMIC_RELAXED, __HIP_MEMORY_SCOPE_SYSTEM);
+    } else (void)__hip_atomic_fetch_add((gu32*)&ctl->entered, 1u, RLX_AGENT);
+    if (n_carry && __hip_atomic_load((const gu32*)&ctl->adopt, RLX_AGENT) < n_carry)
+      for (;;) {
+        const unsigned k = __hip_atomic_fetch_add((gu32*)&ctl->adopt, 1u, RLX_AGENT);
+        if (k >= n_carry) break;
+        const unsigned g = __hip_atomic_fetch_add((gu32*)&ctl->pub, 1u, RLX_AGENT);
+        __hip_atomic_store((gu32*)reinterpret_cast<unsigned*>(ring + (size_t)(g & 7u) * ring_cap + (g >> 3)), prev->carry[k], RLX_AGENT);
+      }
+  }
+  return ctl->n_live + n_carry;
 }
 
 #define NDT_CTX_PARAMS(i) const float* __restrict__ src##i, size_t pitch##i, PairState* st##i, const GridDesc* __restrict__ gd##i, const BitWord* __restrict__ words##i, \
@@ -221,7 +269,13 @@
   const gu32* ringx = (const gu32*)reinterpret_cast<const unsigned*>(ring + (size_t)x * ring_cap);
   const gu32* fin_p = (const gu32*)&ctl->fin;
   gu32* pos_p = (gu32*)&ctl->pos[x * ASYNC_POS_STRIDE];
-  const unsigned n_live = ctl->n_live;
+  const unsigned n_live = async_enter(ctl, ring, ring_cap);
+  if (n_live == 0u) {
+    unsigned first = 1u;
+    if (lane == 0) first = __hip_atomic_fetch_add((gu32*)&ctl->adopt, 1u, RLX_AGENT);
+    if (__builtin_amdgcn_readfirstlane(first) == 0u) async_report(ctl, 0u, lane);
+    return;
+  }
   const int I = items_per_pair;
   const int CLAIM = K == 1 ? ASYNC_CLAIM(1) : (claim_items == 2 ? 2 : 1);
   const int Iu = I / CLAIM;
@@ -259,7 +313,7 @@
               int ws = (int)__hip_atomic_load(slot, RLX_AGENT);
               unsigned lag = 0;
               while (ws < 0 && ++lag <= ASYNC_SPIN_LIMIT) { __builtin_amdgcn_s_sleep(2); ws = (int)__hip_atomic_load(slot, RLX_AGENT); }
-              if (ws < 0) { give_up(); w = -2; break; }
+              if (ws < 0) { give_up(); w = -3; break; }
               w = ws; sp = q; st = 1;
               break;
             }
@@ -267,7 +321,7 @@
         }
         __builtin_amdgcn_s_sleep(32);
         if (t < ring_cap) w = (int)__hip_atomic_load(ringx + t, RLX_AGENT);
-        if (++spins > ASYNC_SPIN_LIMIT) { give_up(); w = -2; break; }
+        if (++spins > ASYNC_SPIN_LIMIT) { give_up(); w = -3; break; }
       }
     }
     w = __builtin_amdgcn_readfirstlane(w);
@@ -281,11 +335,11 @@
   int tw = -1;
   if (lane == 0 && (int)(pos / (unsigned)Iu) < ring_cap) tw = (int)__hip_atomic_load(ringx + pos / (unsigned)Iu, RLX_AGENT);
   tw = wait_ticket(pos, tw);
-  if (tw < 0) return;
+  if (tw < 0) { if (tw == -3) async_report(ctl, n_live, lane); return; }
   unsigned pose_w = sweep_pose_words(NDT_CTX_SEL(st, tw >> ASYNC_CTX_SHIFT) + (tw & ((1 << ASYNC_CTX_SHIFT) - 1)));
 #pragma unroll 1
   for (;;) {
-    if (x == 0 && pos == debug_abort_pos) { if (lane == 0) give_up(); break; }
+    if (x == 0 && pos == debug_abort_pos) { if (lane == 0) give_up(); async_report(ctl, n_live, lane); break; }
     const int rem = (int)(pos % (unsigned)Iu) * CLAIM;
     TL_STAMP(10);
     const int ci = tw >> ASYNC_CTX_SHIFT;
@@ -333,7 +387,7 @@
     }
     if (ntw < 0) {
       ntw = wait_ticket(npos, ntw);
-      if (ntw < 0) break;
+      if (ntw < 0) { if (ntw == -3) async_report(ctl, n_live, lane); break; }
       npose = sweep_pose_words(NDT_CTX_SEL(st, ntw >> ASYNC_CTX_SHIFT) + (ntw & ((1 << ASYNC_CTX_SHIFT) - 1)));
     }
     tw = ntw; pos = npos; pose_w = npose;
diff --git a/lv_slam_amd/csrc/ndt_build.hpp b/lv_slam_amd/csrc/ndt_build.hpp
--- a/lv_slam_amd/csrc/ndt_build.hpp
+++ b/lv_slam_amd/csrc/ndt_build.hpp
@@ -450,7 +450,7 @@
   }
 }
 
-__global__ void __launch_bounds__(256) k_voxels(const GridDesc* __restrict__ gd, const double* __restrict__ sums,
+__global__ void __launch_bounds__(256, 6) k_voxels(const GridDesc* __restrict__ gd, const double* __restrict__ sums,
                                                  VoxelRec* recs, int* vox_n, double eig_mult, int pca, double* icov64, int* kd_weight,
                                                  VoxelRecF* recs_fast ) {
   const int b = blockIdx.y;
diff --git a/lv_slam_amd/csrc/ndt_engine.hpp b/lv_slam_amd/csrc/ndt_engine.hpp
--- a/lv_slam_amd/csrc/ndt_engine.hpp
+++ b/lv_slam_amd/csrc/ndt_engine.hpp
@@ -25,6 +25,7 @@
   void* pose_next = nullptr; size_t pose_cap_next = 0; int pose_base_next = 0, pose_stride_next = 1;
   long long next_id = 0, launches = 0, counted = 0;
   long long recovered_upto = -1;
+  static constexpr int SETS = 4;
   DevBuf<AsyncCtl> d_ctl;
   DevBuf<int> d_ring;
   DevBuf<CtxStat> d_stat;
@@ -32,7 +33,7 @@
   bool lean = false;
   bool reserve_given = false;
   int last_reserve = 0, last_slots = 0;
-  HipEvent ev_built[ASYNC_MAX_CTX], ev_launched[EV], ev_prepared[EV]; bool prep_first = true;
+  HipEvent ev_built[ASYNC_MAX_CTX];
   PinBuf<volatile StreamStatus> h_status; StreamStatus* d_status = nullptr;
   StreamCtx ctx[ASYNC_MAX_CTX];
 };
diff --git a/lv_slam_amd/csrc/ndt_host_stream.hpp b/lv_slam_amd/csrc/ndt_host_stream.hpp
--- a/lv_slam_amd/csrc/ndt_host_stream.hpp
+++ b/lv_slam_amd/csrc/ndt_host_stream.hpp
@@ -77,9 +77,6 @@
     if (ss.reserve_wg > 0 && !ss.build_stream) {
       if (ss.build_stream.create() != hipSuccess) return MI355NDT_ERR_HIP;
       for (auto& ev : ss.ev_built) if (ev.create() != hipSuccess) return MI355NDT_ERR_HIP;
-      for (auto& ev : ss.ev_launched) if (ev.create() != hipSuccess) return MI355NDT_ERR_HIP;
-      for (auto& ev : ss.ev_prepared) if (ev.create() != hipSuccess) return MI355NDT_ERR_HIP;
-      if (const char* pf = std::getenv("MI355NDT_STREAM_PREP_FIRST")) ss.prep_first = std::atoi(pf) != 0;
     }
     rc = mi355ndt_set_stream(e, ss.reserve_wg > 0 ? ss.build_stream : h->stream);
     if (rc) return rc;
@@ -100,21 +97,24 @@
       { h->err = "stream_begin: allocation failed"; return MI355NDT_ERR_HIP; }
     if (h->prof) (void)mi355ndt_profile_enable(e, 1);
   }
-  if (ss.d_ctl.realloc_exact(2) != hipSuccess || hipMemsetAsync(ss.d_ctl, 0, 2 * sizeof(AsyncCtl), h->stream) != hipSuccess ||
+  if (ss.d_ctl.realloc_exact(StreamState::SETS) != hipSuccess || hipMemsetAsync(ss.d_ctl, 0, StreamState::SETS * sizeof(AsyncCtl), h->stream) != hipSuccess ||
       ss.h_status.realloc_exact(StreamState::EV, hipHostMallocMapped | hipHostMallocCoherent) != hipSuccess ||
       !(ss.d_status = ss.h_status.dev())) return MI355NDT_ERR_HIP;
   memset((void*)ss.h_status.p, 0, StreamState::EV * sizeof(StreamStatus));
-  if (h->d_atab.reserve(1) != hipSuccess) return MI355NDT_ERR_HIP;
-  if (!ss.sync_only && ss.d_ring.realloc_exact((size_t)8 * ss.ring_cap) != hipSuccess) { (void)hipGetLastError(); ss.sync_only = true; }
+  if (h->d_atab.reserve(StreamState::SETS) != hipSuccess) return MI355NDT_ERR_HIP;
+  if (!ss.sync_only && ss.d_ring.realloc_exact((size_t)StreamState::SETS * 8 * ss.ring_cap) != hipSuccess) { (void)hipGetLastError(); ss.sync_only = true; }
   if (ss.build_stream) HIPCHK(h, hipStreamSynchronize(ss.build_stream));
   HIPCHK(h, hipStreamSynchronize(h->stream));
   h->ss = std::move(session);
   return MI355NDT_OK;
 }
 
+static int stream_wait_launch(mi355ndt_handle* h, long long j);
 static int stream_launch(mi355ndt_handle* h, int new_ci, int n_new) {
   StreamState& ss = *h->ss;
   hipStream_t s = h->stream;
+  const long long j = ss.launches;
+  if (j >= StreamState::SETS - 1) { const int rcw = stream_wait_launch(h, j - (StreamState::SETS - 1)); if (rcw) return rcw; }
   SweepConst sc;
   make_sweep_const(h, sc);
   AsyncLaunch L;
@@ -132,7 +132,6 @@
     for (int a = 1; a <= ahead; a++) mf = mf || c == (new_ci + a) % ss.nctx;
     L.tab.c[c].must_finish = mf ? 1 : 0;
   }
-  const long long j = ss.launches;
   L.new_ci = flush ? 0 : new_ci; L.n_new = flush ? 0 : n_new;
   if (!flush) {
     mi355ndt_handle* e = ss.ctx[new_ci].e.get();
@@ -140,8 +139,10 @@
     L.active_list = e->d_active_list; L.sweep_ctl = nullptr; L.done_new = &ss.d_stat[new_ci].done;
     L.pose_new = ss.ctx[new_ci].d_pose; L.pose_cap = ss.ctx[new_ci].pose_cap;
   }
-  L.tab_dev = h->d_atab; L.ring = ss.d_ring; L.ring_cap = ss.ring_cap;
-  L.ctl = ss.d_ctl + (j & 1); L.prev = ss.drop_carry ? nullptr : ss.d_ctl + ((j + 1) & 1);
+  const int set = (int)(j % StreamState::SETS), slot = (int)(j % StreamState::EV);
+  L.tab_dev = h->d_atab + set; L.ring = ss.d_ring + (size_t)set * 8 * ss.ring_cap; L.ring_cap = ss.ring_cap;
+  L.ctl = ss.d_ctl + set; L.prev = ss.drop_carry ? nullptr : ss.d_ctl + (int)((j + StreamState::SETS - 1) % StreamState::SETS);
+  L.report = ss.d_status + slot; L.stat = ss.d_stat; L.seq = (unsigned)(j + 1);
   L.items_per_pair = ss.items; L.stop_thresh = flush ? 0 : (ss.thresh_given ? ss.thresh : std::min(ss.thresh, n_new / 4)); L.debug_abort_pos = h->debug_abort_pos; L.debug_ring_mask = h->debug_ring_mask;
   if (!flush) {
     const mi355ndt_handle* e = ss.ctx[new_ci].e.get();
@@ -152,19 +153,20 @@
   L.reserve_wg = flush ? 0 : ss.reserve_wg;
   if (L.lean && !flush && !ss.reserve_given && ss.reserve_wg > 0) L.reserve_wg = LEAN_RESERVE_WG;
   if (L.lean) L.reserve_wg = std::min(L.reserve_wg, launch_slots(h, sc, false, true) / 2) & ~7;
-  L.ev_prepared = (ss.reserve_wg > 0 && ss.prep_first) ? ss.ev_prepared[j % StreamState::EV] : nullptr;
   L.claim_items = (sc.K == 7 && L.stop_thresh > 0) ? 2 : 1;
   h->ev_last_fresh = false;
-  if (!flush && ss.reserve_wg > 0) HIPCHK(h, hipStreamWaitEvent(s, ss.ev_built[new_ci], 0));
-  L.stamp_end = (!flush && h->prof) ? &ss.d_status[j % StreamState::EV].build_t1 : nullptr;
-  int rc = launch_async(h, sc, L);
+  L.stamp_end = (!flush && h->prof) ? &ss.d_status[slot].build_t1 : nullptr;
+  int rc = async_prepare(h, L, flush ? s : ss.ctx[new_ci].e->stream);
   if (rc) return rc;
+  if (!flush && ss.reserve_wg > 0) {
+    HIPCHK(h, hipEventRecord(ss.ev_built[new_ci], ss.ctx[new_ci].e->stream));
+    HIPCHK(h, hipStreamWaitEvent(s, ss.ev_built[new_ci], 0));
+  }
+  rc = async_fire(h, sc, L, false);
+  if (rc) return rc;
+  HIPCHK(h, hipGetLastError());
   ss.drop_carry = false;
   if (!flush) { ss.last_reserve = L.reserve_wg; ss.last_slots = h->last_async_grid; }
-  const int slot = (int)(j % StreamState::EV);
-  k_stream_status<<<1, 64, 0, s>>>(L.ctl, ss.d_stat, reinterpret_cast<volatile unsigned*>(ss.d_status + slot), (unsigned)(j + 1));
-  HIPCHK(h, hipGetLastError());
-  if (ss.reserve_wg > 0) HIPCHK(h, hipEventRecord(ss.ev_launched[slot], s));
   ss.launches++;
   h->P.stream_launches++;
   return MI355NDT_OK;
@@ -184,9 +186,10 @@
   for (; ss.counted <= j; ss.counted++) {
     volatile StreamStatus* c = ss.h_status + (ss.counted % StreamState::EV);
     h->P.stream_carried += c->susp;
-    const unsigned long long b0 = c->build_t0, b1 = c->build_t1;
+    const unsigned long long b0 = c->build_t0, b1 = c->build_t1, l0 = c->launch_t0, l1 = c->launch_t1;
     if (b0 && b1 > b0) { h->P.build_ms += (double)(b1 - b0) * 1e-5; h->P.build_launches++; }
-    c->build_t0 = 0; c->build_t1 = 0;
+    if (l0 && l1 > l0) { h->P.sweep_ms += (double)(l1 - l0) * 1e-5; h->P.sweep_launches++; }
+    c->build_t0 = 0; c->build_t1 = 0; c->launch_t0 = 0; c->launch_t1 = 0;
   }
   return MI355NDT_OK;
 }
@@ -239,13 +242,10 @@
   memcpy(S.h_in, tc, (size_t)n_pairs * sizeof(int));
   memcpy(S.h_in + ss.max_pairs, scnt, (size_t)n_pairs * sizeof(int));
   memcpy(S.h_in + 2 * (size_t)ss.max_pairs, guesses, (size_t)n_pairs * 16 * sizeof(float));
-  if (ss.reserve_wg > 0 && ss.prep_first && ss.launches >= 1)
-    HIPCHK(h, hipStreamWaitEvent(e->stream, ss.ev_prepared[(ss.launches - 1) % StreamState::EV], 0));
-  else if (ss.reserve_wg > 0 && ss.launches >= 2)
-    HIPCHK(h, hipStreamWaitEvent(e->stream, ss.ev_launched[(ss.launches - 2) % StreamState::EV], 0));
   k_stream_inputs<<<1, 1024, 0, e->stream>>>(S.h_in_dev, reinterpret_cast<unsigned*>(S.d_in.p), (unsigned)(2 * (size_t)ss.max_pairs + (size_t)n_pairs * 16),
                                             e->d_word_off, (unsigned)(2 + 6 * (size_t)e->cap_pairs),
-                                            h->prof ? &ss.d_status[ss.launches % StreamState::EV].build_t0 : nullptr);
+                                            h->prof ? &ss.d_status[ss.launches % StreamState::EV].build_t0 : nullptr,
+                                            (ss.reserve_wg > 0 && ss.launches >= 1) ? &ss.d_ctl[(ss.launches - 1) % StreamState::SETS].entered : nullptr);
   e->word_off_cleared = true;
   e->build_stamped = h->prof;
   e->counts_preloaded = true; e->up_src_cnt.clear(); e->up_tgt_cnt.clear();
@@ -255,7 +255,6 @@
   rc = mi355ndt_batch_build_targets(e);
   if (rc) { h->err = e->err; return rc; }
   if (!(e->plan_cb > 0 && e->plan_words > 0)) stream_learn_plan(ss, e);
-  if (ss.reserve_wg > 0) HIPCHK(h, hipEventRecord(ss.ev_built[ci], e->stream));
   stream_geometry(ss, e);
   gauss_constants3(h->prm.outlier_ratio, h->prm.resolution, h->gauss_last);
   S.busy = true;
diff --git a/lv_slam_amd/csrc/ndt_host_sweep.hpp b/lv_slam_amd/csrc/ndt_host_sweep.hpp
--- a/lv_slam_amd/csrc/ndt_host_sweep.hpp
+++ b/lv_slam_amd/csrc/ndt_host_sweep.hpp
@@ -157,10 +157,10 @@
   AsyncTab* tab_dev = nullptr; int* ring = nullptr; int ring_cap = 0; AsyncCtl* ctl = nullptr; const AsyncCtl* prev = nullptr;
   int items_per_pair = 0, stop_thresh = 0; unsigned debug_abort_pos = 0xFFFFFFFFu, debug_ring_mask = 0xFFu;
   unsigned long long* stamp_end = nullptr;
+  StreamStatus* report = nullptr; const CtxStat* stat = nullptr; unsigned seq = 0;
   int claim_items = 1;
   int reserve_wg = 0;
   bool lean = false;
-  hipEvent_t ev_prepared = nullptr;
 };
 #define NDT_CTX_ARGS(i) L.tab.c[i].src, L.tab.c[i].pitch, L.tab.c[i].st, L.tab.c[i].gd, L.tab.c[i].words, L.tab.c[i].recs, L.tab.c[i].partials, L.tab.c[i].src_cnt, \
                         L.tab.c[i].arrived, L.tab.c[i].cent
@@ -182,22 +182,27 @@
   h->last_async_wpe = SweepTune<PCA, K, ORD, LEAN>::WPE; h->last_async_grid = (int)grid.x;
   return MI355NDT_OK;
 }
-static int launch_async(mi355ndt_handle* h, const SweepConst& sc, const AsyncLaunch& L) {
-  hipStream_t s = h->stream;
-  {
-    const size_t n = std::max(std::max(std::max((size_t)8 * L.ring_cap, (size_t)L.n_new * ASYNC_ARR_STRIDE), sizeof(AsyncCtl) / sizeof(unsigned)), (size_t)L.pose_cap);
-    k_async_prepare<<<(unsigned)((n + 255) / 256), 256, 0, s>>>(L.tab, L.tab_dev, L.new_ci, L.n_new, L.st_new, L.guess_new, L.src_cnt_new, L.gd_new, L.arrived_new,
-                                                               L.active_list, L.sweep_ctl, L.ring, L.ring_cap, L.ctl, L.prev, L.done_new, L.pose_new, L.pose_cap, L.stamp_end);
-    if (L.ev_prepared) HIPCHK(h, hipEventRecord(L.ev_prepared, s));
-  }
-  if (h->prof) HIPCHK(h, ev_begin(h, h->ev_sweep));
+static int async_prepare(mi355ndt_handle* h, const AsyncLaunch& L, hipStream_t s) {
+  const size_t n = std::max(std::max(std::max((size_t)8 * L.ring_cap, (size_t)L.n_new * ASYNC_ARR_STRIDE), sizeof(AsyncCtl) / sizeof(unsigned)), (size_t)L.pose_cap);
+  k_async_prepare<<<(unsigned)((n + 255) / 256), 256, 0, s>>>(L.tab, L.tab_dev, L.new_ci, L.n_new, L.st_new, L.guess_new, L.src_cnt_new, L.gd_new, L.arrived_new,
+                                                             L.active_list, L.sweep_ctl, L.ring, L.ring_cap, L.ctl, L.prev, L.done_new, L.pose_new, L.pose_cap, L.stamp_end,
+                                                             L.report, L.stat, L.seq, h->prof ? 1u : 0u);
+  HIPCHK(h, hipGetLastError());
+  return MI355NDT_OK;
+}
+static int async_fire(mi355ndt_handle* h, const SweepConst& sc, const AsyncLaunch& L, bool events) {
+  if (h->prof && events) HIPCHK(h, ev_begin(h, h->ev_sweep));
   const int rc = dispatch_sweep(sc.pca != 0, sc.K, sweep_ord(h, sc), SWEEP_IT_BATCH, [&](auto P, auto KK, auto O, auto) {
     if constexpr (lean_exists(decltype(P)::value, decltype(KK)::value, decltype(O)::value))
       if (L.lean) return launch_async_t<false, 7, decltype(O)::value, true>(h, sc, L);
     return launch_async_t<decltype(P)::value, decltype(KK)::value, decltype(O)::value>(h, sc, L);
   });
-  if (h->prof) HIPCHK(h, ev_end(h, h->ev_sweep));
+  if (h->prof && events) HIPCHK(h, ev_end(h, h->ev_sweep));
   return rc;
+}
+static int launch_async(mi355ndt_handle* h, const SweepConst& sc, const AsyncLaunch& L) {
+  const int rc = async_prepare(h, L, h->stream);
+  return rc ? rc : async_fire(h, sc, L, true);
 }
 static int async_ring_cap(const mi355ndt_handle* h, long long pairs) {
   const long long cap = (pairs * ((long long)h->prm.max_iterations + 4) + 7) / 8 + 1;
```

After: 70760, median of 6. No clear change (+1.0%).
